# IONIQ6000/av1-go

Hardware: AMD Instinct MI355X
Metric: encoded 4K30 frames/sec (whole node) at fixed QP; PSNR-Y delta vs libaom (higher is better)
Workload: dtype u16

## Files before the change

### av1-go_amd/csrc/av1_entropy_kernels.hip

```cpp
#include <string.h>
#include <vector>
#include "av1_ops_cdfs.hpp"
#include "av1_ops32.hpp"
#include "av1mi_internal.hpp"

namespace av1mi {
using namespace av1ops;

struct Av1EntLaunch {
  FrameView fv;
  int nframes, sbr_n, sbc_n;
  BlockInfo *info;
  op_t *ops; uint32_t ops_cap;
  uint32_t *grouped; uint32_t grouped_cap;
  uint16_t *slot_total, *slot_base;
  uint16_t *rec;
  uint32_t *nops;
  uint8_t *slots; uint32_t slot_cap;
  uint32_t *tile_size;
  uint64_t *tile_off;
  uint32_t *status;
  uint8_t *out; uint64_t out_cap;
  const uint16_t *cdf_image; int cdf_words;
  SlotTable tab;
  const uint16_t *cdf_image32; SlotTable tab32;
  const uint8_t *lr_on_frame;
  int sb_rows32, band, nslots;
};

template <int kKey = -1> __device__ __forceinline__ FrameView frame_view(const Av1EntLaunch &L, int f) {
  FrameView v = L.fv;
  const long nb = (long)v.w8 * v.h8;
  if (kKey < 0 ? v.key != 0 : kKey != 0) { v.y_mode += nb * f; v.uv_mode += nb * f; }
  else { v.mv += nb * 2 * f; v.skip += nb * f; }
  v.lev_y += nb * 64 * f; v.lev_u += nb * 16 * f; v.lev_v += nb * 16 * f;
  v.info = L.info + nb * f;
  if (L.lr_on_frame) for (int p = 0; p < 3; p++) v.lr_on[p] = v.lr_on[p] && L.lr_on_frame[f * 3 + p];
  return v;
}

__global__ __launch_bounds__(256) void k_av1_info(Av1EntLaunch L) {
  const long nb = (long)L.fv.w8 * L.fv.h8, i = (long)blockIdx.x * 256 + threadIdx.x;
  if (i >= nb * L.nframes) return;
  const int f = (int)(i / nb), b = (int)(i - (long)f * nb);
  const FrameView v = frame_view(L, f);
  BlockInfo o = {};
  block_summary(v, b, &o);
  if (!v.key) inter_mode_decision(v, b / v.w8, b % v.w8, &o);
  L.info[nb * f + b] = o;
}

constexpr int kReplaySlots = (S_MAX + 1) / 2;
struct TokLds {
  union {
    struct { uint8_t cnt[S_MAX * kBlocksPerTile]; alignas(16) uint8_t mag[kBlocksPerTile * kMagBytes]; } p1;
    uint16_t pos[kReplaySlots * kBlocksPerTile];
  };
  uint16_t total[S_MAX], base[S_MAX];
  ScanTables scan;
};

__global__ __launch_bounds__(64) __attribute__((amdgpu_waves_per_eu(2, 8))) void k_av1_tokens(Av1EntLaunch L) {
  const int tiles = L.sbr_n * L.sbc_n, t = blockIdx.x, f = t / tiles, tt = t - f * tiles, sbr = tt / L.sbc_n, sbc = tt - sbr * L.sbc_n;
  if (sbr < L.sb_rows32) return;
  const FrameView v = frame_view(L, f);
  const int zi = threadIdx.x, nslots = v.key ? S_KEY_END : S_INTER_END;
  __shared__ TokLds S;
  {
    uint32_t *m = reinterpret_cast<uint32_t *>(S.p1.cnt);
    for (int i = zi; i < S_MAX * kBlocksPerTile / 4; i += 64) m[i] = 0;
    if (zi == 0) fill_scan_tables(&S.scan);
  }
  __syncthreads();
  const int below = tiles - L.sb_rows32 * L.sbc_n;
  uint16_t *rec = L.rec + (((size_t)f * below + (tt - (tiles - below))) * kBlocksPerTile + zi) * kBlockRecords;
  const TokScratch ts = { S.p1.mag + zi * kMagBytes, &S.scan };
  Sink k = { rec, S.p1.cnt, zi, 0, 0, false };
  tok_block(v, k, ts, sbr, sbc, zi);
  int x = k.n;
#pragma unroll
  for (int d = 1; d < 64; d <<= 1) {
    const int y = __shfl_up(x, d, 64);
    if (zi >= d) x += y;
  }
  const int total = __shfl(x, 63, 64), first = x - k.n;
  if ((uint32_t)total > L.ops_cap || __any(k.overflow)) {
    if (zi == 0) { atomicOr(L.status, 1u); L.nops[t] = 0; }
    for (int sl = zi; sl < S_MAX; sl += 64) L.slot_total[(size_t)t * S_MAX + sl] = 0;
    return;
  }
  if (zi == 0) L.nops[t] = (uint32_t)total;
  __syncthreads();
  constexpr int kOwn = (S_MAX + 63) / 64;
  uint32_t c[kOwn][kBlocksPerTile / 4];
#pragma unroll
  for (int q = 0; q < kOwn; q++) {
    const int sl = zi + 64 * q;
    int sum = 0;
#pragma unroll
    for (int w = 0; w < kBlocksPerTile / 4; w++) {
      const uint32_t u = sl < nslots ? reinterpret_cast<const uint32_t *>(S.p1.cnt)[sl * (kBlocksPerTile / 4) + w] : 0u;
      c[q][w] = u;
      sum = (int)__builtin_amdgcn_sad_u8(u, 0u, (unsigned)sum);
    }
    if (sl < S_MAX) S.total[sl] = (uint16_t)sum;
  }
  __syncthreads();
  {
    int mine = 0;
    for (int q = 0; q < 4; q++) { const int sl = 4 * zi + q; if (sl < nslots) mine += (S.total[sl] + kListAlign - 1) & ~(kListAlign - 1); }
    int inc = mine;
#pragma unroll
    for (int d = 1; d < 64; d <<= 1) {
      const int y = __shfl_up(inc, d, 64);
      if (zi >= d) inc += y;
    }
    int run = inc - mine;
    for (int q = 0; q < 4; q++) { const int sl = 4 * zi + q; if (sl < nslots) { S.base[sl] = (uint16_t)run; run += (S.total[sl] + kListAlign - 1) & ~(kListAlign - 1); } }
  }
  __syncthreads();
#pragma unroll
  for (int q = 0; q < kOwn; q++) {
    const int sl = zi + 64 * q;
    if (sl >= S_MAX) continue;
    const bool on = sl < nslots;
    L.slot_total[(size_t)t * S_MAX + sl] = on ? S.total[sl] : (uint16_t)0;
    L.slot_base[(size_t)t * S_MAX + sl] = on ? S.base[sl] : (uint16_t)0;
  }
  op_t *list = L.ops + (size_t)t * L.ops_cap;
  uint32_t *grouped = L.grouped + (size_t)t * L.grouped_cap;
#pragma unroll
  for (int half = 0; half < 2; half++) {
    const int lo = half * kReplaySlots, hi = lo + kReplaySlots;
    if (half) __syncthreads();
#pragma unroll
    for (int q = 0; q < kOwn; q++) {
      const int sl = zi + 64 * q;
      if (sl < lo || sl >= hi || sl >= nslots) continue;
      int run = S.base[sl];
#pragma unroll
      for (int w = 0; w < kBlocksPerTile / 4; w++) {
        const uint32_t u = c[q][w];
        const int p0 = run, p1 = p0 + (int)(u & 0xFF), p2 = p1 + (int)((u >> 8) & 0xFF), p3 = p2 + (int)((u >> 16) & 0xFF);
        run = p3 + (int)(u >> 24);
        uint32_t *d = reinterpret_cast<uint32_t *>(S.pos + (sl - lo) * kBlocksPerTile + 4 * w);
        d[0] = (uint32_t)p0 | ((uint32_t)p1 << 16); d[1] = (uint32_t)p2 | ((uint32_t)p3 << 16);
      }
    }
    __syncthreads();
    __threadfence_block();
    replay_block<kBlocksPerTile>(rec, k.nrec, S.pos, zi, first, list, grouped, lo, hi, half == 0);
  }
}

struct Wave32 {
  template <class T> using Var = LaneVar<T, 1>;
  template <class F> __device__ __forceinline__ void each(F f) { f((int)threadIdx.x); __syncthreads(); }
  __device__ __forceinline__ int scan(Var<int> &v) {
    const int lane = (int)threadIdx.x, x = v.v[0];
    int inc = x;
#pragma unroll
    for (int d = 1; d < 64; d <<= 1) {
      const int y = __shfl_up(inc, d, 64);
      if (lane >= d) inc += y;
    }
    v.v[0] = inc - x;
    return __shfl(inc, 63, 64);
  }
  __device__ __forceinline__ int first(Var<int> &v) { return __shfl(v.v[0], 0, 64); }
};
__global__ __launch_bounds__(64) void k_av1_tokens32(Av1EntLaunch L) {
  __shared__ Tile32Mem S;
  const int tiles = L.sbr_n * L.sbc_n, band = L.sb_rows32 * L.sbc_n, f = blockIdx.x / band, tt = blockIdx.x - f * band, sbr = tt / L.sbc_n, sbc = tt - sbr * L.sbc_n;
  const size_t t = (size_t)f * tiles + tt;
  const FrameView v = frame_view<1>(L, f);
  Wave32 w;
  const int n = tok_tile32(w, S, v, sbr, sbc, L.ops + t * L.ops_cap, L.ops_cap, L.grouped + t * L.grouped_cap, L.slot_total + t * S_MAX, L.slot_base + t * S_MAX);
  if (threadIdx.x == 0) {
    if (n < 0) atomicOr(L.status, 1u);
    L.nops[t] = n < 0 ? 0u : (uint32_t)n;
  }
}

__global__ __launch_bounds__(64) void k_av1_chains(Av1EntLaunch L, int ntiles_all, int ngroups) {
  const int xcd = blockIdx.x & 7, j = blockIdx.x >> 3, nslots = L.nslots;
  const int g = (j / nslots) * 8 + xcd, sl = j - (j / nslots) * nslots, lane = threadIdx.x, t = g * 64 + lane;
  if (g >= ngroups) return;
  __shared__ __attribute__((aligned(16))) uint16_t s_big[64 * 16];
  const int n = L.tab.nsym[sl], off = L.tab.off[sl];
  int cnt = 0, base = 0;
  bool mine = t < ntiles_all;
  if (mine && L.band) { const int tiles = L.sbr_n * L.sbc_n, sbr = (t % tiles) / L.sbc_n; mine = (sbr < L.sb_rows32) == (L.band == 1); }
  if (mine) { cnt = L.slot_total[(size_t)t * S_MAX + sl]; base = L.slot_base[(size_t)t * S_MAX + sl]; }
  if (!__any(cnt > 0)) return;
  const size_t tt = t < ntiles_all ? (size_t)t : 0;
  op_t *list = L.ops + tt * L.ops_cap;
  const uint32_t *grouped = L.grouped + tt * L.grouped_cap + base;
  if (n <= 4) {
    const uint32_t *iw = reinterpret_cast<const uint32_t *>(L.cdf_image) + (off >> 1);
    uint64_t cdf = (uint64_t)iw[0] | ((uint64_t)iw[1] << 32);
    const uint4 *g4 = reinterpret_cast<const uint4 *>(grouped);
    const uint4 z = make_uint4(0, 0, 0, 0);
    uint4 c0 = cnt > 0 ? g4[0] : z, c1 = cnt > 4 ? g4[1] : z, c2 = cnt > 8 ? g4[2] : z, c3 = cnt > 12 ? g4[3] : z;
    auto four = [&](const uint4 &v, int e) {
      if (e < cnt) list[v.x >> 4] = small_step(cdf, (int)(v.x & 15), n);
      if (e + 1 < cnt) list[v.y >> 4] = small_step(cdf, (int)(v.y & 15), n);
      if (e + 2 < cnt) list[v.z >> 4] = small_step(cdf, (int)(v.z & 15), n);
      if (e + 3 < cnt) list[v.w >> 4] = small_step(cdf, (int)(v.w & 15), n);
    };
#pragma unroll 1
    for (int e = 0; e < cnt; e += 16) {
      const uint4 *nx = g4 + (e >> 2) + 4;
      const uint4 n0 = e + 16 < cnt ? nx[0] : z, n1 = e + 20 < cnt ? nx[1] : z, n2 = e + 24 < cnt ? nx[2] : z, n3 = e + 28 < cnt ? nx[3] : z;
      four(c0, e); four(c1, e + 4); four(c2, e + 8); four(c3, e + 12);
      c0 = n0; c1 = n1; c2 = n2; c3 = n3;
    }
  } else {
    uint16_t *cdf = s_big + lane * 16;
    {
      const uint4 *iw = reinterpret_cast<const uint4 *>(L.cdf_image + off);
      uint4 *d = reinterpret_cast<uint4 *>(cdf);
      d[0] = iw[0];
      d[1] = n > 8 ? iw[1] : make_uint4(0, 0, 0, 0);
    }
#pragma unroll 1
    for (int e = 0; e < cnt; e++) {
      const uint32_t v = grouped[e];
      const int s = (int)(v & 15);
      list[v >> 4] = s >= kSplitHorz ? split_tuple(cdf, s) : big_step(cdf, s, n);
    }
  }
}

constexpr int kRingOps = 64, kLaneWords = kRingOps * 2 + Coder::kStage + 8;

__global__ __launch_bounds__(64) void k_av1_code(Av1EntLaunch L, int ntiles_all) {
  __shared__ __attribute__((aligned(16))) uint16_t s_lane[64 * kLaneWords];
  const int lane = threadIdx.x, t = blockIdx.x * 64 + lane;
  const bool live = t < ntiles_all;
  uint32_t *ring = reinterpret_cast<uint32_t *>(s_lane + lane * kLaneWords);
  Coder c;
  c.init(L.slots + (size_t)(live ? t : 0) * L.slot_cap, (int)L.slot_cap, s_lane + lane * kLaneWords + kRingOps * 2);
  const int n = live ? (int)L.nops[t] : 0;
  const uint4 *ops4 = reinterpret_cast<const uint4 *>(L.ops + (size_t)(live ? t : 0) * L.ops_cap);
  uint4 r0, r1, r2, r3, r4, r5, r6, r7;
  r0 = r1 = r2 = r3 = r4 = r5 = r6 = r7 = make_uint4(0, 0, 0, 0);
  int w = 0;
  bool pend = false;
  auto request = [&]() {
    const uint4 *p = ops4 + (w >> 2);
    if (w < n) r0 = p[0];
    if (w + 4 < n) r1 = p[1];
    if (w + 8 < n) r2 = p[2];
    if (w + 12 < n) r3 = p[3];
    if (w + 16 < n) r4 = p[4];
    if (w + 20 < n) r5 = p[5];
    if (w + 24 < n) r6 = p[6];
    if (w + 28 < n) r7 = p[7];
    pend = w < n;
  };
  auto take = [&]() {
    uint4 *q = reinterpret_cast<uint4 *>(ring + (w & 32));
    q[0] = r0; q[1] = r1; q[2] = r2; q[3] = r3; q[4] = r4; q[5] = r5; q[6] = r6; q[7] = r7;
    w += 32;
  };
  request();
  if (pend) { take(); request(); }
  int i = 0, lit_left = 0;
  uint32_t op = ring[0], op_next = ring[1], op_next2 = ring[2];
  for (;;) {
    if (!__any(lit_left > 0 || i < n)) break;
    if (__any((pend && w - i < 24) || c.ns >= Coder::kStage - 8)) {
      if (pend && w - i <= 32) { take(); request(); }
      c.spill();
    }
#pragma unroll
    for (int q = 0; q < 8; q++) {
      if (lit_left > 0 || i < n) {
        const uint32_t fetched = ring[(i + 3) & (kRingOps - 1)];
        uint32_t tup = op;
        if (lit_left == 0 && (op >> 31)) lit_left = (int)((op >> 27) & 15);
        if (lit_left > 0) {
          lit_left--;
          tup = (op >> lit_left) & 1 ? (1u << 19) | (256u << 9) : (2u << 19) | (512u << 9) | 256u;
        }
        c.encode_tuple(tup);
        if (lit_left == 0) { i++; op = op_next; op_next = op_next2; op_next2 = fetched; }
      }
    }
  }
  if (!live) return;
  int sz = n ? c.finish() : -1;
  if (sz < 0) { if (n) atomicOr(L.status, 2u); sz = 0; }
  L.tile_size[t] = (uint32_t)sz;
}

__global__ __launch_bounds__(1024) void k_av1_scan(Av1EntLaunch L, int ntiles_all) {
  __shared__ uint64_t part[1024];
  const int tid = threadIdx.x, per = (ntiles_all + 1023) / 1024, i0 = tid * per, i1 = min(i0 + per, ntiles_all);
  uint64_t s = 0;
  for (int i = i0; i < i1; i++) s += L.tile_size[i];
  part[tid] = s;
  __syncthreads();
  for (int d = 1; d < 1024; d <<= 1) {
    const uint64_t y = tid >= d ? part[tid - d] : 0;
    __syncthreads();
    part[tid] += y;
    __syncthreads();
  }
  uint64_t run = part[tid] - s;
  for (int i = i0; i < i1; i++) { L.tile_off[i] = run; run += L.tile_size[i]; }
  if (tid == 1023) {
    L.tile_off[ntiles_all] = part[1023];
    if (part[1023] > L.out_cap) atomicOr(L.status, 4u);
  }
}
__global__ __launch_bounds__(64) void k_av1_gather(Av1EntLaunch L) {
  const int t = blockIdx.x;
  const uint32_t n = L.tile_size[t];
  const uint64_t off = L.tile_off[t];
  if (off + n > L.out_cap) return;
  const uint8_t *src = L.slots + (size_t)t * L.slot_cap;
  uint8_t *dst = L.out + off;
  const uint32_t head = min(n, (uint32_t)((16 - (reinterpret_cast<uintptr_t>(dst) & 15)) & 15)), body = (n - head) >> 4, tail0 = head + (body << 4);
  if (threadIdx.x < head) dst[threadIdx.x] = src[threadIdx.x];
  for (uint32_t i = threadIdx.x; i < body; i += 64) {
    uint4 v;
    __builtin_memcpy(&v, src + head + 16 * i, 16);
    *reinterpret_cast<uint4 *>(dst + head + 16 * i) = v;
  }
  if (tail0 + threadIdx.x < n) dst[tail0 + threadIdx.x] = src[tail0 + threadIdx.x];
}

hipError_t launch_av1_front(av1mi_ctx *ctx, const Av1EntLaunch &L, hipStream_t s) {
  const long nb = (long)L.fv.w8 * L.fv.h8 * L.nframes;
  const int ntiles_all = L.sbr_n * L.sbc_n * L.nframes, ngroups = (ntiles_all + 63) / 64;
  ProfToken t = ctx_prof_begin(ctx, AV1MI_K_ENTROPY_TOKENS, s);
  hipLaunchKernelGGL(k_av1_info, dim3((unsigned)((nb + 255) / 256)), dim3(256), 0, s, L);
  if (L.sb_rows32 < L.sbr_n) hipLaunchKernelGGL(k_av1_tokens, dim3((unsigned)ntiles_all), dim3(64), 0, s, L);
  if (L.sb_rows32) hipLaunchKernelGGL(k_av1_tokens32, dim3((unsigned)(L.sb_rows32 * L.sbc_n * L.nframes)), dim3(64), 0, s, L);
  ctx_prof_end(ctx, t, s);
  t = ctx_prof_begin(ctx, AV1MI_K_ENTROPY_CHAINS, s);
  Av1EntLaunch C = L;
  C.nslots = L.fv.key ? S_KEY_END : S_INTER_END; C.band = L.sb_rows32 ? 2 : 0;
  if (L.sb_rows32 < L.sbr_n) hipLaunchKernelGGL(k_av1_chains, dim3((unsigned)(((ngroups + 7) / 8) * 8 * C.nslots)), dim3(64), 0, s, C, ntiles_all, ngroups);
  if (L.sb_rows32) {
    C.nslots = K_END; C.band = 1; C.tab = L.tab32; C.cdf_image = L.cdf_image32;
    hipLaunchKernelGGL(k_av1_chains, dim3((unsigned)(((ngroups + 7) / 8) * 8 * C.nslots)), dim3(64), 0, s, C, ntiles_all, ngroups);
  }
  ctx_prof_end(ctx, t, s);
  return hipGetLastError();
}
hipError_t launch_av1_back(av1mi_ctx *ctx, const Av1EntLaunch &L, hipStream_t s) {
  const int ntiles_all = L.sbr_n * L.sbc_n * L.nframes;
  ProfToken t = ctx_prof_begin(ctx, AV1MI_K_ENTROPY, s);
  hipLaunchKernelGGL(k_av1_code, dim3((unsigned)((ntiles_all + 63) / 64)), dim3(64), 0, s, L, ntiles_all);
  ctx_prof_end(ctx, t, s);
  t = ctx_prof_begin(ctx, AV1MI_K_ENTROPY_PACK, s);
  hipLaunchKernelGGL(k_av1_scan, dim3(1), dim3(1024), 0, s, L, ntiles_all);
  hipLaunchKernelGGL(k_av1_gather, dim3((unsigned)ntiles_all), dim3(64), 0, s, L);
  ctx_prof_end(ctx, t, s);
  return hipGetLastError();
}

}

struct av1mi_av1ent_state {
  void *info = nullptr, *ops[2] = { nullptr, nullptr }, *nops[2] = { nullptr, nullptr }, *grouped = nullptr, *slot_tb = nullptr, *rec = nullptr, *slots = nullptr, *tile_off = nullptr, *status = nullptr;
  size_t info_b = 0, ops_b[2] = { 0, 0 }, nops_b[2] = { 0, 0 }, grouped_b = 0, slot_tb_b = 0, rec_b = 0, slots_b = 0, off_b = 0;
  hipEvent_t lists_ready[2] = { nullptr, nullptr }, lists_free[2] = { nullptr, nullptr };
  bool free_recorded[2] = { false, false };
  unsigned long jobs = 0;
  av1mi::Av1EntLaunch pending[2];
  uint64_t *pending_total[2] = { nullptr, nullptr };
  bool pending_valid[2] = { false, false };
  size_t last_tiles = 0;
  uint16_t *d_image[2][4] = {};
  uint16_t *d_image32[4] = {};
  av1ops::SlotTable tab32;
  int image_words[2] = { 0, 0 };
  av1ops::SlotTable tab[2];
};

namespace {
int grow(av1mi_ctx *ctx, void **p, size_t *have, size_t need) {
  if (*have >= need) return AV1MI_OK;
  if (*p) (void)hipFree(*p);
  *p = nullptr; *have = 0;
  if (hipMalloc(p, need) != hipSuccess) return av1mi::ctx_fail(ctx, AV1MI_E_NOMEM, "AV1 entropy scratch: hipMalloc(%zu) failed", need);
  *have = need;
  return AV1MI_OK;
}
}

extern "C" {

uint32_t av1mi_av1_entropy_ops_per_tile(void) { return 32768; }
uint32_t av1mi_av1_entropy_slot_bytes(void) { return 16384; }

}

int av1mi::av1_entropy_front(av1mi_ctx *ctx, const av1mi_av1_entropy_job *j, hipStream_t front, int *ticket) {
  if (!ctx || !ticket) return AV1MI_E_INVAL;
  *ticket = -1;
  if (!j) return av1mi::ctx_fail(ctx, AV1MI_E_INVAL, "null job");
  if (hipSetDevice(av1mi::ctx_device(ctx)) != hipSuccess) return av1mi::ctx_fail(ctx, AV1MI_E_DEVICE, "hipSetDevice failed");
  if (j->width <= 0 || j->height <= 0 || (j->width & 7) || (j->height & 7) || j->width > 4096 || j->height > 4096)
    return av1mi::ctx_fail(ctx, AV1MI_E_INVAL, "frame %dx%d must be a multiple of 8, at most 4096x4096", j->width, j->height);
  if (j->nframes < 0 || j->nframes > 4096 || j->base_q_idx < 1 || j->base_q_idx > 255) return av1mi::ctx_fail(ctx, AV1MI_E_INVAL, "bad nframes / base_q_idx");
  const void *need[] = { j->d_lev_y, j->d_lev_u, j->d_lev_v, j->d_out, j->d_tile_size, j->d_total, j->key ? (const void *)j->d_modes_y : (const void *)j->d_mvs,
                         j->key ? (const void *)j->d_modes_uv : (const void *)j->d_skip };
  for (const void *p : need) if (!p) return av1mi::ctx_fail(ctx, AV1MI_E_INVAL, "null device pointer");
  if (j->nframes == 0) return AV1MI_OK;
  av1mi_av1ent_state *st = av1mi::ctx_av1ent(ctx);
  if (!st) return av1mi::ctx_fail(ctx, AV1MI_E_NOMEM, "AV1 entropy state");
  const int key = j->key ? 1 : 0, qcat = av1ops::q_category(j->base_q_idx);
  if (!st->d_image[key][qcat]) {
    av1ops::SlotTable tab;
    const std::vector<uint16_t> img = av1ops::default_slot_image(key != 0, qcat, &tab);
    st->tab[key] = tab; st->image_words[key] = tab.words;
    if (hipMalloc((void **)&st->d_image[key][qcat], img.size() * 2) != hipSuccess ||
        hipMemcpy(st->d_image[key][qcat], img.data(), img.size() * 2, hipMemcpyHostToDevice) != hipSuccess)
      return av1mi::ctx_fail(ctx, AV1MI_E_DEVICE, "uploading the default CDF image failed");
  }
  if (j->key_rows32 && (!key || (j->key_rows32 & 63) || j->key_rows32 > j->height || (j->width & 31)))
    return av1mi::ctx_fail(ctx, AV1MI_E_INVAL, "key_rows32 %d: whole superblock rows of a key frame whose width is a multiple of 32", j->key_rows32);
  if (j->key_rows32 && !st->d_image32[qcat]) {
    const std::vector<uint16_t> img = av1ops::default_slot_image_k32(qcat, &st->tab32);
    if (hipMalloc((void **)&st->d_image32[qcat], img.size() * 2) != hipSuccess ||
        hipMemcpy(st->d_image32[qcat], img.data(), img.size() * 2, hipMemcpyHostToDevice) != hipSuccess)
      return av1mi::ctx_fail(ctx, AV1MI_E_DEVICE, "uploading the default CDF image failed");
  }
  av1mi::Av1EntLaunch L;
  memset(&L, 0, sizeof(L));
  L.sb_rows32 = j->key_rows32 / 64;
  if (j->key_rows32) { L.tab32 = st->tab32; L.cdf_image32 = st->d_image32[qcat]; }
  L.fv.w8 = j->width / 8; L.fv.h8 = j->height / 8; L.fv.key = key;
  L.fv.y_mode = j->d_modes_y; L.fv.uv_mode = j->d_modes_uv; L.fv.mv = j->d_mvs; L.fv.skip = j->d_skip;
  L.fv.lev_y = j->d_lev_y; L.fv.lev_u = j->d_lev_u; L.fv.lev_v = j->d_lev_v;
  for (int p = 0; p < 3; p++) {
    L.fv.lr_on[p] = j->lr_on[p] != 0;
    const int vh = j->visible_height ? j->visible_height : j->height, vw = j->visible_width ? j->visible_width : j->width;
    const int ph = p ? (vh + 1) / 2 : vh, pw = p ? (vw + 1) / 2 : vw;
    L.fv.lr_rows[p] = (ph + 32) / 64 > 1 ? (ph + 32) / 64 : 1; L.fv.lr_cols[p] = (pw + 32) / 64 > 1 ? (pw + 32) / 64 : 1;
  }
  memcpy(L.fv.lr_unit[0], j->lr_unit_y, 8); memcpy(L.fv.lr_unit[1], j->lr_unit_uv, 8);
  L.nframes = j->nframes; L.sbr_n = (L.fv.h8 + 7) / 8; L.sbc_n = (L.fv.w8 + 7) / 8;
  const size_t nb = (size_t)L.fv.w8 * L.fv.h8 * j->nframes, nt = (size_t)L.sbr_n * L.sbc_n * j->nframes;
  L.ops_cap = av1mi_av1_entropy_ops_per_tile(); L.slot_cap = av1mi_av1_entropy_slot_bytes();
  L.grouped_cap = L.ops_cap + av1ops::kListAlign * av1ops::S_MAX;
  const int par = (int)(st->jobs++ & 1);
  st->last_tiles = nt;
  int rc;
  if ((rc = grow(ctx, &st->info, &st->info_b, nb * sizeof(av1ops::BlockInfo))) ||
      (rc = grow(ctx, &st->ops[par], &st->ops_b[par], nt * L.ops_cap * sizeof(av1ops::op_t))) || (rc = grow(ctx, &st->nops[par], &st->nops_b[par], nt * 4)) ||
      (rc = grow(ctx, &st->grouped, &st->grouped_b, nt * L.grouped_cap * sizeof(uint32_t))) ||
      (rc = grow(ctx, &st->slot_tb, &st->slot_tb_b, nt * av1ops::S_MAX * 4)) ||
      (rc = grow(ctx, &st->rec, &st->rec_b, (size_t)(L.sbr_n - L.sb_rows32) * L.sbc_n * j->nframes * av1ops::kBlocksPerTile * av1ops::kBlockRecords * sizeof(uint16_t))) ||
      (rc = grow(ctx, &st->slots, &st->slots_b, nt * L.slot_cap)) || (rc = grow(ctx, &st->tile_off, &st->off_b, (nt + 1) * 8)))
    return rc;
  L.info = (av1ops::BlockInfo *)st->info; L.ops = (av1ops::op_t *)st->ops[par]; L.nops = (uint32_t *)st->nops[par]; L.grouped = (uint32_t *)st->grouped;
  L.slot_total = (uint16_t *)st->slot_tb; L.slot_base = L.slot_total + nt * av1ops::S_MAX; L.rec = (uint16_t *)st->rec; L.slots = (uint8_t *)st->slots;
  L.tile_off = (uint64_t *)st->tile_off;
  L.tile_size = j->d_tile_size; L.out = j->d_out; L.out_cap = j->out_cap;
  L.status = (uint32_t *)(j->d_total + 1);
  L.cdf_image = st->d_image[key][qcat]; L.cdf_words = st->image_words[key]; L.tab = st->tab[key];
  L.lr_on_frame = j->d_lr_on;
#define E_HIP(call) do { const hipError_t e_ = (call); if (e_ != hipSuccess) return av1mi::ctx_fail(ctx, AV1MI_E_DEVICE, "%s: %s", #call, hipGetErrorString(e_)); } while (0)
  for (hipEvent_t *ev : { &st->lists_ready[par], &st->lists_free[par] }) if (!*ev) E_HIP(hipEventCreateWithFlags(ev, hipEventDisableTiming));
  if (st->free_recorded[par]) E_HIP(hipStreamWaitEvent(front, st->lists_free[par], 0));
  E_HIP(hipMemsetAsync(j->d_total, 0, 16, front));
  E_HIP(av1mi::launch_av1_front(ctx, L, front));
  E_HIP(hipEventRecord(st->lists_ready[par], front));
  st->pending[par] = L; st->pending_total[par] = j->d_total; st->pending_valid[par] = true;
  *ticket = par;
  return AV1MI_OK;
}

int av1mi::av1_entropy_back(av1mi_ctx *ctx, int ticket, hipStream_t back) {
  if (!ctx || ticket < 0 || ticket > 1) return AV1MI_E_INVAL;
  av1mi_av1ent_state *st = av1mi::ctx_av1ent(ctx);
  if (!st || !st->pending_valid[ticket]) return av1mi::ctx_fail(ctx, AV1MI_E_INVAL, "no entropy job pending under this ticket");
  const av1mi::Av1EntLaunch &L = st->pending[ticket];
  const size_t nt = (size_t)L.sbr_n * L.sbc_n * L.nframes;
  E_HIP(hipStreamWaitEvent(back, st->lists_ready[ticket], 0));
  E_HIP(av1mi::launch_av1_back(ctx, L, back));
  E_HIP(hipMemcpyAsync(st->pending_total[ticket], L.tile_off + nt, 8, hipMemcpyDeviceToDevice, back));
  E_HIP(hipEventRecord(st->lists_free[ticket], back)); st->free_recorded[ticket] = true;
  st->pending_valid[ticket] = false;
#undef E_HIP
  return AV1MI_OK;
}

int av1mi::av1_entropy_submit(av1mi_ctx *ctx, const av1mi_av1_entropy_job *j, hipStream_t front, hipStream_t back) {
  int ticket = -1;
  const int rc = av1_entropy_front(ctx, j, front, &ticket);
  if (rc != AV1MI_OK || ticket < 0) return rc;
  return av1_entropy_back(ctx, ticket, back);
}

extern "C" {

int av1mi_av1_entropy_encode_on(av1mi_ctx *ctx, const av1mi_av1_entropy_job *j, void *stream_handle) {
  if (!ctx) return AV1MI_E_INVAL;
  hipStream_t s = stream_handle ? (hipStream_t)stream_handle : av1mi::ctx_stream(ctx);
  return av1mi::av1_entropy_submit(ctx, j, s, s);
}

int av1mi_av1_entropy_encode(av1mi_ctx *ctx, const av1mi_av1_entropy_job *j) { return av1mi_av1_entropy_encode_on(ctx, j, nullptr); }

int av1mi_av1_entropy_last_list_words(av1mi_ctx *ctx, uint64_t *words) {
  if (!ctx || !words) return AV1MI_E_INVAL;
  *words = 0;
  av1mi_av1ent_state *st = av1mi::ctx_av1ent(ctx);
  if (!st || !st->jobs || !st->last_tiles) return AV1MI_OK;
  if (hipSetDevice(av1mi::ctx_device(ctx)) != hipSuccess || hipDeviceSynchronize() != hipSuccess) return av1mi::ctx_fail(ctx, AV1MI_E_DEVICE, "synchronising failed");
  std::vector<uint32_t> n(st->last_tiles);
  if (hipMemcpy(n.data(), st->nops[(st->jobs - 1) & 1], n.size() * 4, hipMemcpyDeviceToHost) != hipSuccess) return av1mi::ctx_fail(ctx, AV1MI_E_DEVICE, "reading the list sizes failed");
  for (uint32_t v : n) *words += v;
  return AV1MI_OK;
}

}

namespace av1mi {
void av1ent_free(av1mi_av1ent_state *st) {
  if (!st) return;
  for (void *p : { st->info, st->ops[0], st->ops[1], st->nops[0], st->nops[1], st->grouped, st->slot_tb, st->rec, st->slots, st->tile_off }) if (p) (void)hipFree(p);
  for (hipEvent_t ev : { st->lists_ready[0], st->lists_ready[1], st->lists_free[0], st->lists_free[1] }) if (ev) (void)hipEventDestroy(ev);
  for (auto &k : st->d_image) for (uint16_t *p : k) if (p) (void)hipFree(p);
  for (uint16_t *p : st->d_image32) if (p) (void)hipFree(p);
  delete st;
}
av1mi_av1ent_state *av1ent_new() { return new (std::nothrow) av1mi_av1ent_state(); }
}
```

### av1-go_amd/csrc/av1_ops.hpp

```cpp
#pragma once
#include <stdint.h>

#if defined(__HIPCC__)
#include <hip/hip_runtime.h>
#define AV1_HD __host__ __device__ inline
#define AV1_UNROLL _Pragma("unroll")
#define AV1_NOUNROLL _Pragma("unroll 1")
#else
#define AV1_HD inline
#define AV1_UNROLL
#define AV1_NOUNROLL
#endif

namespace av1ops {

typedef uint16_t __attribute__((may_alias)) u16a;
typedef uint32_t __attribute__((may_alias)) u32a;
typedef uint64_t __attribute__((may_alias)) u64a;

enum Slot : int {
  S_SKIP = 0,
  S_PART8 = S_SKIP + 3,
  S_PART16 = S_PART8 + 1,
  S_PART32 = S_PART16 + 4,
  S_PART64 = S_PART32 + 4,
  S_USE_WIENER = S_PART64 + 4,
  S_TXB_SKIP_Y = S_USE_WIENER + 1,
  S_TXB_SKIP_C = S_TXB_SKIP_Y + 1,
  S_EOB64_Y = S_TXB_SKIP_C + 3,
  S_EOB16_C = S_EOB64_Y + 1,
  S_EOBX_Y = S_EOB16_C + 1,
  S_EOBX_C = S_EOBX_Y + 5,
  S_DC_SIGN_Y = S_EOBX_C + 3,
  S_DC_SIGN_C = S_DC_SIGN_Y + 3,
  S_BASE_EOB_Y = S_DC_SIGN_C + 3,
  S_BASE_EOB_C = S_BASE_EOB_Y + 4,
  S_BASE_Y = S_BASE_EOB_C + 4,
  S_BASE_C = S_BASE_Y + 26,
  S_BR_Y = S_BASE_C + 26,
  S_BR_C = S_BR_Y + 21,
  S_COMMON_END = S_BR_C + 21,
  S_KF_Y_MODE = S_COMMON_END,
  S_UV_MODE = S_KF_Y_MODE + 25,
  S_ANGLE = S_UV_MODE + 13,
  S_INTRA_TX = S_ANGLE + 8,
  S_KEY_END = S_INTRA_TX + 13,
  S_IS_INTER = S_COMMON_END,
  S_SINGLE_REF = S_IS_INTER + 4,
  S_NEW_MV = S_SINGLE_REF + 6,
  S_ZERO_MV = S_NEW_MV + 6,
  S_REF_MV = S_ZERO_MV + 1,
  S_DRL = S_REF_MV + 6,
  S_MV_JOINT = S_DRL + 3,
  S_MV_COMP = S_MV_JOINT + 1,
  S_INTER_TX = S_MV_COMP + 32,
  S_INTER_END = S_INTER_TX + 1,
  S_MAX = S_KEY_END > S_INTER_END ? S_KEY_END : S_INTER_END
};
enum { MVC_CLASS = 0, MVC_CLASS0 = 1, MVC_CLASS0_FR = 2, MVC_SIGN = 4, MVC_BITS = 5, MVC_FR = 15 };

struct BandSlots {
  int use_wiener, kf_y_mode, uv_mode, angle;
  int txb_skip_y, txb_skip_c, eob_y, eob_c, eobx_y, eobx_c, dc_sign_y, dc_sign_c, base_eob_y, base_eob_c, base_y, base_c, br_y, br_c;
  int eob_y_n, eob_c_n;
};
constexpr BandSlots kSlots8 = { S_USE_WIENER, S_KF_Y_MODE, S_UV_MODE, S_ANGLE, S_TXB_SKIP_Y, S_TXB_SKIP_C, S_EOB64_Y, S_EOB16_C, S_EOBX_Y,
                                S_EOBX_C, S_DC_SIGN_Y, S_DC_SIGN_C, S_BASE_EOB_Y, S_BASE_EOB_C, S_BASE_Y, S_BASE_C, S_BR_Y, S_BR_C, 7, 5 };

template <const BandSlots &B> AV1_HD int coeff_nsym(int s) {
  if (s < B.txb_skip_y || s >= B.br_c + 21) return 0;
  if (s == B.eob_y) return B.eob_y_n;
  if (s == B.eob_c) return B.eob_c_n;
  return s < B.base_eob_y ? 2 : s < B.base_y ? 3 : 4;
}
AV1_HD int slot_nsym(int s, bool key) {
  if (const int n = coeff_nsym<kSlots8>(s)) return n;
  if (s < S_PART8) return 2;
  if (s < S_PART16) return 4;
  if (s < S_USE_WIENER) return 10;
  if (s < S_COMMON_END) return 2;
  if (key) {
    if (s < S_UV_MODE) return 13;
    if (s < S_ANGLE) return 14;
    if (s < S_INTRA_TX) return 7;
    return 7;
  }
  if (s < S_MV_JOINT) return 2;
  if (s == S_MV_JOINT) return 4;
  if (s < S_INTER_TX) {
    const int k = (s - S_MV_COMP) & 15;
    return k == MVC_CLASS ? 11 : (k == MVC_CLASS0_FR || k == MVC_CLASS0_FR + 1 || k == MVC_FR) ? 4 : 2;
  }
  return 16;
}
AV1_HD int q_category(int base_q_idx) { return base_q_idx <= 20 ? 0 : base_q_idx <= 60 ? 1 : base_q_idx <= 120 ? 2 : 3; }
AV1_HD int slot_words(int nsym) { return nsym <= 4 ? 4 : nsym <= 8 ? 8 : 16; }

typedef uint32_t op_t;
struct SlotTable { uint16_t off[S_MAX]; uint8_t nsym[(S_MAX + 3) & ~3]; int words; };
AV1_HD op_t op_lit(int n, unsigned v) { return (op_t)(0x80000000u | ((unsigned)n << 27) | (v & 0x7FFu)); }
AV1_HD op_t make_tuple(uint32_t fl, uint32_t fh, int s, int n) { return (op_t)(((unsigned)(n - s) << 19) | ((fl >> 6) << 9) | (fh >> 6)); }
enum { kBlocksPerTile = 64, kSplitHorz = 14, kSplitVert = 15, kListAlign = 4, kBlockRecords = 1024 };

struct Sink {
  uint16_t *rec;
  uint8_t *cnt;
  int zi, nrec, n;
  bool overflow;
  AV1_HD void put(unsigned r) { if (nrec < kBlockRecords) rec[nrec] = (uint16_t)r; else overflow = true; nrec++; n++; }
  AV1_HD void sym(int slot, int s) {
    put(((unsigned)slot << 4) | (unsigned)s);
    uint8_t &c = cnt[slot * kBlocksPerTile + zi];
    if (c == 255) overflow = true; else c++;
  }
  AV1_HD void split(int kind, int slot) { sym(slot, kind ? kSplitVert : kSplitHorz); }
  AV1_HD void lit(unsigned v, int nbits) {
    while (nbits > 11) { nbits -= 11; put(0x8000u | (11u << 11) | ((v >> nbits) & 0x7FFu)); }
    if (nbits > 0) put(0x8000u | ((unsigned)nbits << 11) | (v & ((1u << nbits) - 1u)));
  }
};
AV1_HD int group_positions(const uint8_t *cnt_slot, uint16_t *pos_slot, int base) {
  int run = base;
  for (int b = 0; b < kBlocksPerTile; b++) { const int c = cnt_slot[b]; pos_slot[b] = (uint16_t)run; run += c; }
  return run - base;
}
template <int kBlocks>
AV1_HD void replay_block(const uint16_t *rec, int nrec, uint16_t *pos, int blk, int first, op_t *list, uint32_t *grouped, int slot_lo = 0,
                         int slot_hi = 1 << 16, bool literals = true) {
  int n = first;
  for (int i0 = 0; i0 < nrec; i0 += 8) {
    struct alignas(16) R8 { uint32_t w[4]; } q = *reinterpret_cast<const R8 *>(rec + i0);
    AV1_UNROLL
    for (int j = 0; j < 8; j++, n++) {
      if (i0 + j >= nrec) break;
      const unsigned r = (q.w[j >> 1] >> (16 * (j & 1))) & 0xFFFFu;
      if (r & 0x8000u) { if (literals) list[n] = op_lit((int)((r >> 11) & 15), r & 0x7FFu); }
      else {
        const int sl = (int)(r >> 4);
        if (sl >= slot_lo && sl < slot_hi) { uint16_t &p = pos[(sl - slot_lo) * kBlocks + blk]; grouped[p] = ((uint32_t)n << 4) | (r & 15u); p++; }
      }
    }
  }
}

struct BlockInfo { uint8_t cul[3], dc[3], mode, flags; uint8_t num, drl; int16_t px, py; uint8_t pad[2]; };
struct FrameView {
  int w8, h8;
  int key;
  const uint8_t *y_mode, *uv_mode;
  const int16_t *mv;
  const uint8_t *skip;
  const int16_t *lev_y, *lev_u, *lev_v;
  const BlockInfo *info;
  int lr_on[3];
  int8_t lr_unit[2][8];
  int lr_rows[3], lr_cols[3];
};

AV1_HD int iabs(int v) { return v < 0 ? -v : v; }
AV1_HD int imin(int a, int b) { return a < b ? a : b; }
AV1_HD int imax(int a, int b) { return a > b ? a : b; }
AV1_HD int ilog2(unsigned v) { return 31 - __builtin_clz(v | 1u); }
AV1_HD unsigned morton8(unsigned x, unsigned y) {
  unsigned m = 0;
  for (int i = 0; i < 3; i++) m |= ((x >> i) & 1u) << (2 * i) | ((y >> i) & 1u) << (2 * i + 1);
  return m;
}
AV1_HD void demorton8(unsigned k, int *bx, int *by) {
  int x = 0, y = 0;
  for (int i = 0; i < 3; i++) { x |= ((k >> (2 * i)) & 1) << i; y |= ((k >> (2 * i + 1)) & 1) << i; }
  *bx = x; *by = y;
}

AV1_HD void block_summary(const FrameView &f, int b, BlockInfo *o) {
  const int16_t *p[3] = { f.lev_y + (long)b * 64, f.lev_u + (long)b * 16, f.lev_v + (long)b * 16 };
  const bool skip = !f.key && f.skip[b];
  for (int pl = 0; pl < 3; pl++) {
    int cul = 0;
    const int n = pl ? 16 : 64;
    for (int i = 0; i < n; i++) cul += iabs(p[pl][i]);
    o->cul[pl] = skip ? 0 : (uint8_t)imin(cul, 63);
    o->dc[pl] = skip ? 0 : (uint8_t)(p[pl][0] < 0 ? 1 : p[pl][0] > 0 ? 2 : 0);
  }
}

struct MvCand { int16_t x, y; int weight; };
struct MvStack { MvCand st[8]; int num, new_ctx, ref_ctx; };

AV1_HD void mv_stack(const FrameView &f, int r8, int c8, bool use_flags, MvStack *S) {
  const int r0 = r8 & ~7, c0 = c8 & ~7, r1 = imin(r0 + 8, f.h8), c1 = imin(c0 + 8, f.w8);
  int num = 0, new_count = 0;
  bool found = false;
  MvCand *st = S->st;
  auto add = [&](int r, int c, bool count_new) {
    if (r < r0 || r >= r1 || c < c0 || c >= c1) return;
    const int nb = r * f.w8 + c;
    const int16_t mx = f.mv[2 * nb], my = f.mv[2 * nb + 1];
    if (count_new && use_flags && (f.info[nb].flags & 1)) new_count++;
    found = true;
    int i = 0;
    for (; i < num; i++) if (st[i].x == mx && st[i].y == my) break;
    if (i < num) st[i].weight += 4;
    else if (num < 8) { st[num].x = mx; st[num].y = my; st[num].weight = 4; num++; }
  };
  add(r8 - 1, c8, true);
  const bool above0 = found; found = false;
  add(r8, c8 - 1, true);
  const bool left0 = found; found = false;
  {
    const int tr = r8 - 1, tc = c8 + 1;
    if (tr >= r0 && tc < c1 && morton8(tc & 7, tr & 7) < morton8(c8 & 7, r8 & 7)) add(tr, tc, true);
  }
  bool above = above0 || found; found = false;
  const int close = (above ? 1 : 0) + (left0 ? 1 : 0);
  const int num_nearest = num, num_new = new_count;
  for (int i = 0; i < num_nearest; i++) st[i].weight += 640;
  add(r8 - 1, c8 - 1, false);
  above = above || found; found = false;
  bool left = left0;
  add(r8 - 2, c8, false); above = above || found; found = false;
  add(r8, c8 - 2, false); left = left || found; found = false;
  add(r8 - 3, c8, false); above = above || found; found = false;
  add(r8, c8 - 3, false); left = left || found; found = false;
  const int total = (above ? 1 : 0) + (left ? 1 : 0);
  for (int pass = 0; pass < 2; pass++) {
    const int a = pass ? num_nearest : 0, bnd = pass ? num : num_nearest;
    for (int len = bnd; len > a;) {
      int nr = a;
      for (int i = a + 1; i < len; i++)
        if (st[i - 1].weight < st[i].weight) { const MvCand t = st[i - 1]; st[i - 1] = st[i]; st[i] = t; nr = i; }
      len = nr;
    }
  }
  if (close == 0) { S->new_ctx = imin(total, 1); S->ref_ctx = total; }
  else if (close == 1) { S->new_ctx = 3 - imin(num_new, 1); S->ref_ctx = 2 + total; }
  else { S->new_ctx = 5 - imin(num_new, 1); S->ref_ctx = 5; }
  const int mi_r = r8 * 2, mi_c = c8 * 2, border = 128 + 2 * 4 * 8;
  const int top = -(mi_r * 32) - border, bottom = (f.h8 * 2 - 2 - mi_r) * 32 + border;
  const int lft = -(mi_c * 32) - border, right = (f.w8 * 2 - 2 - mi_c) * 32 + border;
  for (int i = 0; i < num; i++) {
    st[i].y = (int16_t)imin(imax(st[i].y, top), bottom);
    st[i].x = (int16_t)imin(imax(st[i].x, lft), right);
  }
  for (int i = num; i < 2; i++) { st[i].x = st[i].y = 0; st[i].weight = 0; }
  S->num = num;
}
AV1_HD void inter_mode_decision(const FrameView &f, int r8, int c8, BlockInfo *o) {
  MvStack S;
  mv_stack(f, r8, c8, false, &S);
  const int b = r8 * f.w8 + c8, mx = f.mv[2 * b], my = f.mv[2 * b + 1];
  int mode = 3, ref_idx = 0;
  if (S.st[0].x == mx && S.st[0].y == my) mode = 0;
  else {
    for (int i = 1; i < imax(S.num, 2) && i < 4; i++)
      if (S.st[i].x == mx && S.st[i].y == my) { mode = 1; ref_idx = i; break; }
    if (mode == 3 && mx == 0 && my == 0) mode = 2;
  }
  if (mode == 3) {
    const int nsel = imin(S.num, 3);
    long best = -1;
    for (int i = 0; i < imax(nsel, 1); i++) {
      const long c = iabs(mx - S.st[i].x) + iabs(my - S.st[i].y);
      if (best < 0 || c < best) { best = c; ref_idx = i; }
    }
  }
  o->mode = (uint8_t)(mode | (ref_idx << 2));
  o->flags = (uint8_t)(mode == 3);
  o->num = (uint8_t)S.num;
  int drl = 0;
  for (int i = 0; i < 4; i++) if (i < imax(S.num, 2) && S.st[i].weight >= 640) drl |= 1 << i;
  o->drl = (uint8_t)drl;
  const int pred = S.num <= 1 ? 0 : ref_idx;
  o->px = S.st[pred].x; o->py = S.st[pred].y;
}

template <class K> AV1_HD void tok_subexp(K &k, int num_syms, int kk, int v) {
  int i = 0, mk = 0;
  for (;;) {
    const int b2 = i ? kk + i - 1 : kk, a = 1 << b2;
    if (num_syms <= mk + 3 * a) {
      const int n = num_syms - mk, x = v - mk, w = ilog2((unsigned)n) + 1, m = (1 << w) - n;
      if (x < m) k.lit((unsigned)x, w - 1);
      else { k.lit((unsigned)((x + m) >> 1), w - 1); k.lit((unsigned)((x + m) & 1), 1); }
      return;
    }
    const int more = v >= mk + a;
    k.lit((unsigned)more, 1);
    if (!more) { k.lit((unsigned)(v - mk), b2); return; }
    i++; mk += a;
  }
}
AV1_HD int tok_recenter(int r, int v) { return v > 2 * r ? v : v >= r ? 2 * (v - r) : 2 * (r - v) - 1; }
template <class K> AV1_HD void tok_signed_subexp_ref(K &k, int v, int low, int high, int kk, int r) {
  const int mx = high - low;
  v -= low; r -= low;
  tok_subexp(k, mx, kk, (r << 1) <= mx ? tok_recenter(r, v) : tok_recenter(mx - 1 - r, mx - 1 - v));
}
template <const BandSlots &B, class K> AV1_HD void tok_lr(const FrameView &f, K &k, int sbr, int sbc) {
  const int mi_r = sbr * 16, mi_c = sbc * 16;
  for (int p = 0; p < 3; p++) {
    if (!f.lr_on[p]) continue;
    const int ss = p ? 1 : 0, us = 64;
    const int row0 = (mi_r * (4 >> ss) + us - 1) / us, row1 = imin(((mi_r + 16) * (4 >> ss) + us - 1) / us, f.lr_rows[p]);
    const int col0 = (mi_c * (4 >> ss) + us - 1) / us, col1 = imin(((mi_c + 16) * (4 >> ss) + us - 1) / us, f.lr_cols[p]);
    const int8_t *u = f.lr_unit[p ? 1 : 0];
    for (int ur = row0; ur < row1; ur++)
      for (int uc = col0; uc < col1; uc++) {
        k.sym(B.use_wiener, u[0] == 1);
        if (u[0] != 1) continue;
        const int kmin[3] = { -5, -23, -17 }, kmax[3] = { 10, 8, 46 }, kk[3] = { 1, 2, 3 }, mid[3] = { 3, -7, 15 };
        for (int pass = 0; pass < 2; pass++)
          for (int j = p ? 1 : 0; j < 3; j++) tok_signed_subexp_ref(k, u[1 + pass * 3 + j], kmin[j], kmax[j] + 1, kk[j], mid[j]);
      }
  }
}
template <const BandSlots &B, class K> AV1_HD void tok_kf_modes(K &k, int ym, int uvm, int above, int left) {
  static const uint8_t kCtx[13] = { 0, 1, 2, 3, 4, 4, 4, 4, 3, 0, 1, 2, 0 };
  k.sym(B.kf_y_mode + kCtx[above] * 5 + kCtx[left], ym);
  if (ym >= 1 && ym <= 8) k.sym(B.angle + ym - 1, 3);
  k.sym(B.uv_mode + ym, uvm);
  if (uvm >= 1 && uvm <= 8) k.sym(B.angle + uvm - 1, 3);
}
AV1_HD void tok_partition_prefix(const FrameView &f, Sink &k, int sbr, int sbc, int bx, int by) {
  const int mi_rows = f.h8 * 2, mi_cols = f.w8 * 2;
  for (int bsize = 64; bsize >= 16; bsize >>= 1) {
    const int n8 = bsize >> 3;
    if ((bx & (n8 - 1)) || (by & (n8 - 1))) continue;
    const int r = (sbr * 8 + by) * 2, c = (sbc * 8 + bx) * 2, half = bsize >> 3;
    const bool has_rows = r + half < mi_rows, has_cols = c + half < mi_cols;
    const bool au = by > 0, al = bx > 0;
    const int slot = (bsize == 16 ? S_PART16 : bsize == 32 ? S_PART32 : S_PART64) + (al ? 2 : 0) + (au ? 1 : 0);
    if (has_rows && has_cols) k.sym(slot, 3);
    else if (has_cols) k.split(0, slot);
    else if (has_rows) k.split(1, slot);
  }
  k.sym(S_PART8, 0);
}

struct ScanTables { uint8_t s4[16], s8[64], i4[16], i8[64]; };
AV1_HD void fill_scan_tables(ScanTables *t) {
  for (int N = 4; N <= 8; N += 4) {
    uint8_t *o = N == 4 ? t->s4 : t->s8;
    int k = 0;
    for (int d = 0; d < 2 * N - 1; d++)
      for (int i = 0; i <= d; i++) {
        const int r = (d & 1) ? i : d - i, c = d - r;
        if (r < N && c < N) o[k++] = (uint8_t)(r * N + c);
      }
    uint8_t *inv = N == 4 ? t->i4 : t->i8;
    for (int i = 0; i < N * N; i++) inv[o[i]] = (uint8_t)i;
  }
}
enum { kMagStride = 10, kMagBytes = 100 };
struct TokScratch { uint8_t *mag; const ScanTables *scan; };

template <int N, bool kBytes = (N <= 8)> struct MagMap;
template <int N> struct MagMap<N, true> {
  enum { LG = N == 4 ? 2 : 3, MS = kMagStride };
  uint8_t *mag;
  const uint8_t *scan, *iscan;
  AV1_HD MagMap(const TokScratch &ts) : mag(ts.mag), scan(N == 4 ? ts.scan->s4 : ts.scan->s8), iscan(N == 4 ? ts.scan->i4 : ts.scan->i8) {}
  AV1_HD int load(const int16_t *lev) {
    for (int i = 0; i < (N + 2) * MS / 4; i++) reinterpret_cast<u32a *>(mag)[i] = 0;
    int eob = 0;
    for (int r = 0; r < N * N / 8; r++) {
      struct alignas(16) L8 { int16_t v[8]; } q = *reinterpret_cast<const L8 *>(lev + 8 * r);
      for (int j = 0; j < 8; j++) {
        const int pos = 8 * r + j, v = q.v[j], a = iabs(v);
        if (v) eob = imax(eob, iscan[pos] + 1);
        mag[(pos >> LG) * MS + (pos & (N - 1))] = (uint8_t)((a > 15 ? 15 : a) | (v < 0 ? 128 : 0));
      }
    }
    return eob;
  }
  AV1_HD int pos(int c) const { return scan[c]; }
  AV1_HD int at(int i) const { return mag[i] & 15; }
  AV1_HD int neg(int p) const { return mag[(p >> LG) * MS + (p & (N - 1))] >> 7; }
};

template <int N, const BandSlots &B, class K>
AV1_HD void tok_coeffs_lead(K &k, bool chroma, int eob, int above_cul, int above_dc, int left_cul, int left_dc, int tx_slot, int tx_sym) {
  k.sym(chroma ? B.txb_skip_c + ((above_cul | above_dc) != 0) + ((left_cul | left_dc) != 0) : B.txb_skip_y, eob == 0);
  if (!eob) return;
  if (tx_slot >= 0) k.sym(tx_slot, tx_sym);
  const int eob_pt = eob < 3 ? eob : ilog2((unsigned)(eob - 1)) + 2;
  k.sym(chroma ? B.eob_c : B.eob_y, eob_pt - 1);
  if (eob_pt >= 3) {
    const int off = eob - ((1 << (eob_pt - 2)) + 1), shift = eob_pt - 3;
    k.sym((chroma ? B.eobx_c : B.eobx_y) + eob_pt - 3, (off >> shift) & 1);
    if (shift > 0) k.lit((unsigned)(off & ((1 << shift) - 1)), shift);
  }
}
template <int N, const BandSlots &B, class K, class M_>
AV1_HD void tok_coeffs_pass1(K &k, const M_ &M, bool chroma, const int16_t *lev, int eob, int c_hi, int c_lo) {
  const int nc = N * N, LG = M.LG, MS = M.MS;
  const int base_eob = chroma ? B.base_eob_c : B.base_eob_y, base = chroma ? B.base_c : B.base_y, br = chroma ? B.br_c : B.br_y;
  for (int c = c_hi; c >= c_lo; c--) {
    const int pos = M.pos(c), row = pos >> LG, col = pos & (N - 1), at = row * MS + col;
    const int m0 = M.at(at), m1 = M.at(at + 1), m2 = M.at(at + 2), mb = M.at(at + MS), md = M.at(at + MS + 1), mbb = M.at(at + 2 * MS);
    int a = m0;
    if (a == 15) a = iabs(lev[pos]);
    if (c == eob - 1) {
      k.sym(base_eob + (c == 0 ? 0 : c <= nc / 8 ? 1 : c <= nc / 4 ? 2 : 3), imin(a, 3) - 1);
    } else {
      const int mm = imin(m1, 3) + imin(mb, 3) + imin(md, 3) + imin(m2, 3) + imin(mbb, 3);
      int bctx = imin((mm + 1) >> 1, 4);
      if (pos == 0) bctx = 0;
      else bctx += row + col < 2 ? 1 : row + col < 4 ? 6 : 21;
      k.sym(base + bctx, imin(a, 3));
    }
    if (a > 2) {
      int mm = m1 + mb + md;
      mm = imin((mm + 1) >> 1, 6);
      const int rctx = pos == 0 ? mm : (row < 2 && col < 2) ? mm + 7 : mm + 14;
      int rem = a - 3;
      for (int i = 0; i < 4; i++) {
        const int q = imin(rem, 3);
        k.sym(br + rctx, q);
        rem -= q;
        if (q < 3) break;
      }
    }
  }
}
template <int N, const BandSlots &B, class K, class M_>
AV1_HD void tok_coeffs_pass2(K &k, const M_ &M, bool chroma, const int16_t *lev, int above_dc, int left_dc, int c_lo, int c_hi) {
  const int LG = M.LG, MS = M.MS;
  for (int c = c_lo; c < c_hi; c++) {
    const int pos = M.pos(c), m = M.at((pos >> LG) * MS + (pos & (N - 1)));
    if (!m) continue;
    const int neg = M.neg(pos);
    if (c == 0) {
      const int sg = (above_dc == 2) - (above_dc == 1) + (left_dc == 2) - (left_dc == 1);
      k.sym((chroma ? B.dc_sign_c : B.dc_sign_y) + (sg < 0 ? 1 : sg > 0 ? 2 : 0), neg);
    } else {
      k.lit((unsigned)neg, 1);
    }
    if (m == 15) {
      const int a = iabs(lev[pos]);
      if (a > 14) {
        const unsigned x = (unsigned)(a - 14);
        const int len = ilog2(x) + 1;
        k.lit(0, len - 1);
        k.lit(x, len);
      }
    }
  }
}
template <int N, const BandSlots &B, class K, class TS>
AV1_HD void tok_coeffs(K &k, const TS &ts, bool chroma, const int16_t *lev, int above_cul, int above_dc, int left_cul, int left_dc, int tx_slot,
                       int tx_sym) {
  MagMap<N> M(ts);
  const int eob = M.load(lev);
  tok_coeffs_lead<N, B>(k, chroma, eob, above_cul, above_dc, left_cul, left_dc, tx_slot, tx_sym);
  if (!eob) return;
  tok_coeffs_pass1<N, B>(k, M, chroma, lev, eob, eob - 1, 0);
  tok_coeffs_pass2<N, B>(k, M, chroma, lev, above_dc, left_dc, 0, eob);
}

AV1_HD void tok_mv_comp(Sink &k, int comp, int diff) {
  const int base = S_MV_COMP + comp * 16;
  k.sym(base + MVC_SIGN, diff < 0);
  const int off = iabs(diff) - 1, cls = (off >> 3) < 2 ? 0 : ilog2((unsigned)(off >> 3));
  k.sym(base + MVC_CLASS, cls);
  if (cls == 0) {
    k.sym(base + MVC_CLASS0, off >> 3);
    k.sym(base + MVC_CLASS0_FR + (off >> 3), (off >> 1) & 3);
  } else {
    const int o = off - (2 << (cls + 2)), d = o >> 3;
    for (int i = 0; i < cls; i++) k.sym(base + MVC_BITS + i, (d >> i) & 1);
    k.sym(base + MVC_FR, (o >> 1) & 3);
  }
}

AV1_HD void tok_block(const FrameView &f, Sink &k, const TokScratch &ts, int sbr, int sbc, int zi) {
  int bx, by;
  demorton8((unsigned)zi, &bx, &by);
  const int r8 = sbr * 8 + by, c8 = sbc * 8 + bx;
  if (r8 >= f.h8 || c8 >= f.w8) return;
  if (zi == 0) tok_lr<kSlots8>(f, k, sbr, sbc);
  tok_partition_prefix(f, k, sbr, sbc, bx, by);
  const int b = r8 * f.w8 + c8;
  const bool au = by > 0, al = bx > 0;
  const BlockInfo zero = {};
  const BlockInfo ia = au ? f.info[b - f.w8] : zero, il = al ? f.info[b - 1] : zero;
  const int skip = f.key ? 0 : f.skip[b];
  k.sym(S_SKIP + (au && !f.key ? f.skip[b - f.w8] : 0) + (al && !f.key ? f.skip[b - 1] : 0), skip);
  int ym = 0;
  if (f.key) {
    ym = f.y_mode[b];
    tok_kf_modes<kSlots8>(k, ym, f.uv_mode[b], au ? f.y_mode[b - f.w8] : 0, al ? f.y_mode[b - 1] : 0);
  } else {
    k.sym(S_IS_INTER + 0, 1);
    const int rctx = (au || al) ? 1 : 0;
    k.sym(S_SINGLE_REF + rctx * 3 + 0, 0);
    k.sym(S_SINGLE_REF + rctx * 3 + 1, 0);
    k.sym(S_SINGLE_REF + rctx * 3 + 2, 0);
    const BlockInfo me = f.info[b];
    const int mode = me.mode & 3, ref_idx = me.mode >> 2, num = me.num;
    const int mx = f.mv[2 * b], my = f.mv[2 * b + 1];
    const int close = (au ? 1 : 0) + (al ? 1 : 0);
    int num_new = (au ? ia.flags & 1 : 0) + (al ? il.flags & 1 : 0);
    if (au && bx < 7 && c8 + 1 < f.w8 && morton8((unsigned)bx + 1, (unsigned)by - 1) < morton8((unsigned)bx, (unsigned)by)) num_new += f.info[b - f.w8 + 1].flags & 1;
    const int new_ctx = close == 0 ? 0 : close == 1 ? 3 - imin(num_new, 1) : 5 - imin(num_new, 1);
    const int ref_ctx = close == 0 ? 0 : close == 1 ? 3 : 5;
    k.sym(S_NEW_MV + new_ctx, mode != 3);
    if (mode != 3) {
      k.sym(S_ZERO_MV, mode != 2);
      if (mode != 2) k.sym(S_REF_MV + ref_ctx, mode == 1);
    }
    auto drl_ctx = [&](int i) {
      const bool a = (me.drl >> i) & 1, c = (me.drl >> (i + 1)) & 1;
      return a && c ? 0 : a ? 1 : !c ? 2 : 0;
    };
    if (mode == 3) {
      for (int i = 0; i < 2; i++)
        if (num > i + 1) {
          k.sym(S_DRL + drl_ctx(i), ref_idx != i);
          if (ref_idx == i) break;
        }
      const int dx = mx - me.px, dy = my - me.py;
      k.sym(S_MV_JOINT, (dx ? 1 : 0) + (dy ? 2 : 0));
      if (dy) tok_mv_comp(k, 0, dy);
      if (dx) tok_mv_comp(k, 1, dx);
    } else if (mode == 1) {
      for (int i = 1; i < 3; i++)
        if (num > i + 1) {
          k.sym(S_DRL + drl_ctx(i), ref_idx != i);
          if (ref_idx == i) break;
        }
    }
  }
  if (skip) return;
  tok_coeffs<8, kSlots8>(k, ts, false, f.lev_y + (long)b * 64, ia.cul[0], ia.dc[0], il.cul[0], il.dc[0], f.key ? S_INTRA_TX + ym : S_INTER_TX, f.key ? 1 : 7);
  AV1_NOUNROLL
  for (int p = 1; p < 3; p++)
    tok_coeffs<4, kSlots8>(k, ts, true, (p == 1 ? f.lev_u : f.lev_v) + (long)b * 16, ia.cul[p], ia.dc[p], il.cul[p], il.dc[p], -1, 0);
}

template <class F> AV1_HD void build_slot_table(int n, F nsym, SlotTable *t) {
  int o = 0;
  for (int s = 0; s < S_MAX; s++) {
    if (s < n) {
      t->nsym[s] = (uint8_t)nsym(s);
      const int w = slot_words(t->nsym[s]), al = w < 8 ? 4 : 8;
      o = (o + al - 1) & ~(al - 1);
      t->off[s] = (uint16_t)o;
      o += w;
    } else { t->nsym[s] = 2; t->off[s] = 0; }
  }
  t->words = (o + 7) & ~7;
}
AV1_HD void build_slot_table(bool key, SlotTable *t) { build_slot_table(key ? S_KEY_END : S_INTER_END, [key](int s) { return slot_nsym(s, key); }, t); }

#ifdef AV1_CODER_STATS
static long long coder_stat_carries = 0;
#endif
struct Coder {
  enum { kStage = 32 };
  uint64_t low;
  uint32_t rng;
  int nb;
  uint8_t *out;
  uint16_t *stage;
  int pos, cap, ns;
  bool overflow;
  AV1_HD void init(uint8_t *o, int c, uint16_t *st) { low = 0; rng = 0x8000; nb = -1; out = o; stage = st; pos = 0; cap = c; ns = 0; overflow = false; }
  AV1_HD void carry_back() {
    for (int k = ns; k-- > 0;) { const uint16_t v = (uint16_t)(stage[k] + 1); stage[k] = v; if (v) return; }
    for (int i = pos; i-- > 0;) if (++out[i] != 0) return;
  }
  AV1_HD bool stage_full() const { return ns >= kStage - 1; }
  AV1_HD void spill() {
    if (pos + 2 * ns > cap) { overflow = true; pos += 2 * ns; ns = 0; return; }
    for (int k = 0; k < ns; k++) { const uint32_t v = stage[k]; *reinterpret_cast<uint16_t *>(out + pos + 2 * k) = (uint16_t)((v >> 8) | (v << 8)); }
    pos += 2 * ns; ns = 0;
  }
  AV1_HD void flush16() {
    nb -= 16;
    const uint32_t w = (uint32_t)(low >> (16 + nb));
    if ((w >> 16) && !overflow) {
#ifdef AV1_CODER_STATS
      coder_stat_carries++;
#endif
      carry_back();
    }
    stage[ns++] = (uint16_t)w;
    low &= ((uint64_t)1 << (16 + nb)) - 1;
  }
  AV1_HD void encode(uint32_t fl, uint32_t fh, int s, int n) {
    const uint32_t r = rng, v = (((r >> 8) * (fh >> 6)) >> 1) + 4u * (uint32_t)(n - 1 - s);
    const uint32_t u = fl < 32768u ? (((r >> 8) * (fl >> 6)) >> 1) + 4u * (uint32_t)(n - s) : r;
    low += r - u;
    const uint32_t nr = u - v;
    const int d = 15 - ilog2(nr);
    rng = nr << d; low <<= d; nb += d;
    if (nb >= 32) flush16();
  }
  AV1_HD void encode_tuple(op_t t) {
    const uint32_t fl6 = (t >> 9) & 1023u, fh6 = t & 511u, dl = (t >> 19) & 31u;
    const uint32_t r = rng, v = (((r >> 8) * fh6) >> 1) + 4u * (dl - 1u);
    const uint32_t u = fl6 < 512u ? (((r >> 8) * fl6) >> 1) + 4u * dl : r;
    low += r - u;
    const uint32_t nr = u - v;
    const int d = 15 - ilog2(nr);
    rng = nr << d; low <<= d; nb += d;
    if (nb >= 32) flush16();
  }
  AV1_HD void bit(int b) { encode(b ? 16384u : 32768u, b ? 0u : 16384u, b, 2); }
  AV1_HD int finish() {
    uint64_t e = ((low + 0x3FFF) & ~(uint64_t)0x3FFF) | 0x4000;
    if (nb >= 0 && (e >> (16 + nb))) { if (!overflow) carry_back(); e &= ((uint64_t)1 << (16 + nb)) - 1; }
    spill();
    int top = 15 + nb;
    while (top >= 14) {
      uint8_t byte = 0;
      for (int q = 7; q >= 0 && top >= 14; q--, top--) byte |= (uint8_t)(((e >> top) & 1) << q);
      if (pos < cap) out[pos] = byte; else overflow = true;
      pos++;
    }
    return overflow ? -1 : pos;
  }
};

AV1_HD uint32_t adapt(uint32_t x, bool below, int rate) {
  const uint32_t m = 0u - (uint32_t)below, d = ((x ^ m) + (m & 32769u)) >> rate;
  return x - ((d ^ m) - m);
}

AV1_HD op_t small_step(uint64_t &w, int s, int n) {
  const uint32_t x0 = (uint32_t)w & 0xFFFFu, x1 = (uint32_t)w >> 16, x2 = (uint32_t)(w >> 32) & 0xFFFFu, cnt = (uint32_t)(w >> 48);
  const uint32_t fl = s == 0 ? 32768u : s == 1 ? x0 : s == 2 ? x1 : x2;
  const uint32_t fh = s == n - 1 ? 0u : s == 0 ? x0 : s == 1 ? x1 : x2;
  const int rate = 3 + (cnt > 15) + (cnt > 31) + (n >= 4 ? 2 : 1);
  const uint32_t y0 = adapt(x0, 0 < s, rate), y1 = adapt(x1, 1 < s, rate), y2 = adapt(x2, 2 < s, rate), ncnt = cnt + (cnt < 32);
  w = (uint64_t)(y0 | (y1 << 16)) | ((uint64_t)(y2 | (ncnt << 16)) << 32);
  return make_tuple(fl, fh, s, n);
}

AV1_HD op_t big_step(uint16_t *v, int s, int n) {
  const int nd = n > 8 ? 8 : 4;
  u32a *d = reinterpret_cast<u32a *>(v);
  uint32_t w[8];
  AV1_UNROLL
  for (int k = 0; k < 8; k++) w[k] = k < nd ? d[k] : 0u;
  const uint32_t fl = s ? v[s - 1] : 32768u, fh = s == n - 1 ? 0u : v[s];
  const uint32_t cnt = (nd == 8 ? w[7] : w[3]) >> 16;
  const int rate = 3 + (cnt > 15) + (cnt > 31) + 2;
  AV1_UNROLL
  for (int k = 0; k < 8; k++) {
    if (k >= nd) continue;
    uint32_t lo = adapt(w[k] & 0xFFFFu, 2 * k < s, rate), hi = adapt(w[k] >> 16, 2 * k + 1 < s, rate);
    if (k == nd - 1) hi = cnt + (cnt < 32);
    d[k] = lo | (hi << 16);
  }
  return make_tuple(fl, fh, s, n);
}

AV1_HD op_t split_tuple(const uint16_t *p, int kind) {
  const uint32_t p1 = p[0] - p[1], p2 = p[1] - p[2], p3 = p[2] - p[3], p4 = p[3] - p[4], p5 = p[4] - p[5], p6 = p[5] - p[6], p7 = p[6] - p[7],
                 p8 = p[7] - p[8], p9 = p[8];
  return make_tuple(kind == kSplitHorz ? p2 + p3 + p4 + p6 + p7 + p9 : p1 + p3 + p4 + p5 + p6 + p8, 0, 1, 2);
}

AV1_HD void run_chain(const uint16_t *init, int n, const uint32_t *g, int cnt, op_t *list) {
  if (n <= 4) {
    uint64_t w = (uint64_t)init[0] | ((uint64_t)init[1] << 16) | ((uint64_t)init[2] << 32) | ((uint64_t)init[3] << 48);
    for (int k = 0; k < cnt; k++) list[g[k] >> 4] = small_step(w, (int)(g[k] & 15), n);
    return;
  }
  alignas(16) uint16_t v[16];
  for (int i = 0; i < 16; i++) v[i] = i < slot_words(n) ? init[i] : 0;
  for (int k = 0; k < cnt; k++) {
    const int s = (int)(g[k] & 15);
    list[g[k] >> 4] = s >= kSplitHorz ? split_tuple(v, s) : big_step(v, s, n);
  }
}

AV1_HD void code_word(Coder &c, op_t e) {
  if (e >> 31) { for (int i = (int)((e >> 27) & 15) - 1; i >= 0; i--) { c.bit((e >> i) & 1); if (c.stage_full()) c.spill(); } }
  else { c.encode_tuple(e); if (c.stage_full()) c.spill(); }
}

}
```

### av1-go_amd/csrc/gop_session.hip

```cpp
#include <math.h>
#include <stdio.h>
#include <stdlib.h>
#include <string.h>
#include <new>
#include <vector>
#include "av1mi_internal.hpp"
#include "quality.hpp"

namespace {

int lf_level_from_q(int ac_q, int bd, bool key) {
  long g;
  if (bd == 8) g = key ? ((long)ac_q * 17563 - 421574 + (1 << 17)) >> 18 : ((long)ac_q * 6017 + 650707 + (1 << 17)) >> 18;
  else g = ((long)ac_q * 20723 + 4060632 + (1 << 19)) >> 20;
  return (int)(g < 0 ? 0 : g > 63 ? 63 : g);
}
void frame_params(int q, int bd, int frame_type, av1mi_frame_params *p) {
  memset(p, 0, sizeof(*p));
  const int ac_q = av1mi_ac_q(q, bd), q8 = ac_q >> (bd - 8);
  p->frame_type = frame_type; p->base_q_idx = q;
  const int lvl = lf_level_from_q(ac_q, bd, frame_type == 0);
  p->lf_level[0] = p->lf_level[1] = p->lf_level[2] = p->lf_level[3] = lvl;
  p->lf_sharpness = 0;
  p->cdef_damping = 3 + (q >> 6);
  {
    const float x = (float)q8, x2 = x * x;
    auto fit = [&](float a, float b, float c, int hi) { const int v = (int)lroundf(x2 * a + x * b + c); return v < 0 ? 0 : v > hi ? hi : v; };
    int y1, y2, c1, c2;
    if (frame_type == 0) {
      y1 = fit(0.0000033731974f, 0.008070594f, 0.0187634f, 15); y2 = fit(0.0000029167343f, 0.0027798624f, 0.0079405f, 3);
      c1 = fit(-0.0000130790995f, 0.012892405f, -0.00748388f, 15); c2 = fit(0.0000032651783f, 0.00035520183f, 0.00228092f, 3);
    } else {
      y1 = fit(-0.0000023593946f, 0.0068615186f, 0.02709886f, 15); y2 = fit(-0.00000057629734f, 0.0013993345f, 0.03831067f, 3);
      c1 = fit(-0.0000007095069f, 0.0034628846f, 0.00887099f, 15); c2 = fit(0.00000023874085f, 0.00028223585f, 0.05576307f, 3);
    }
    p->cdef_y = (uint8_t)(y1 << 2 | y2); p->cdef_uv = (uint8_t)(c1 << 2 | c2);
  }
  p->lr_unit_size = 64;
  static const int8_t wy[8] = { 1, 3, -7, 15, 3, -7, 15, 0 }, wc[8] = { 1, 0, -7, 15, 0, -7, 15, 0 };
  memcpy(p->lr_unit_y, wy, 8); memcpy(p->lr_unit_uv, wc, 8);
}

enum { kSlots = 3, kFallbacksToHostMode = 3 };

struct Plane { int ss = 0, w = 0, h = 0, vw = 0, vh = 0; size_t n = 0, bytes = 0; };

struct Slot {
  void *h_in[3] = { nullptr, nullptr, nullptr }, *d_in[3] = { nullptr, nullptr, nullptr };
  void *d_pre[3] = { nullptr, nullptr, nullptr };
  void *d_src[3] = { nullptr, nullptr, nullptr };
  void *d_lev[3] = { nullptr, nullptr, nullptr }, *h_lev[3] = { nullptr, nullptr, nullptr };
  void *d_modes[2] = { nullptr, nullptr }, *h_modes[2] = { nullptr, nullptr };
  void *d_mv = nullptr, *h_mv = nullptr, *d_skip = nullptr, *h_skip = nullptr;
  hipEvent_t uploaded = nullptr, kernel_done = nullptr, filters_done = nullptr, downloaded = nullptr;
  bool upload_pending = false, kernel_pending = false;
  void *d_lr_on = nullptr, *h_lr_on = nullptr;
  int frame_type = 0;
  int q = 0;
  av1mi_frame_params params{};
  void *h_ent_out = nullptr, *d_tile_size = nullptr, *h_tile_size = nullptr, *d_total = nullptr, *h_total = nullptr;
  hipEvent_t ent_done = nullptr;
  bool ent_pending = false;
  bool symbols_down = false;
  int ent_ticket = -1;
  void *h_quality = nullptr;
  hipEvent_t quality_done = nullptr;
};

}

struct av1mi_gop {
  av1mi_ctx *ctx = nullptr;
  av1mi_gop_config cfg{};
  Plane plane[3];
  size_t nb = 0, bps = 1;
  int fmt = AV1MI_INPUT_PLANAR;
  int stages = 0;
  bool chroma_stage = false, luma_through = false;
  int src_bd = 8;
  av1mi::ScalePlan *scale = nullptr;
  size_t fed_ny = 0;
  size_t in_bytes[3] = {}, pre_bytes[3] = {};
  hipStream_t up = nullptr, down = nullptr;
  Slot slot[kSlots];
  void *d_rec[3] = {}, *d_dbl[3] = {}, *d_cdef[3] = {}, *d_ref[3] = {};
  void *d_mi[3][2] = {};
  int key32 = 0, key_rows32 = 0;
  int key_modes_band = 0, key_modes_stride = 0;
  void *d_cdef_sb[2] = {}, *d_lr[2] = {}, *d_zero_skip = nullptr;
  void *d_lr_scratch = nullptr;
  void *d_me = nullptr;
  void *d_quality_scratch = nullptr;
  int vw = 0, vh = 0;
  int last = 0;
  av1mi_frame_params params[2];
  int next_q = 0;
  int mi_q[3] = {}, cdef_q[2] = {};
  size_t ent_cap = 0; int tiles = 0;
  long submitted = 0, collected = 0;
  long fallbacks = 0;
  bool symbols_always = false;
  int gop_pos = 0;
  bool acquired = false;
  int coder_streams = 0;
  int intra_open_loop = 0;
  std::vector<void *> dev_allocs, host_allocs;
};

namespace {

#define G_HIP(expr)                                                                                          \
  do {                                                                                                       \
    hipError_t e_ = (expr);                                                                                  \
    if (e_ != hipSuccess) return av1mi::ctx_fail(g->ctx, AV1MI_E_DEVICE, "%s: %s", #expr, hipGetErrorString(e_)); \
  } while (0)
#define G_TRY(expr)                              \
  do {                                           \
    int rc_ = (expr);                            \
    if (rc_ != AV1MI_OK) return rc_;             \
  } while (0)

int dev_alloc(av1mi_gop *g, void **p, size_t bytes) {
  G_HIP(hipMalloc(p, bytes ? bytes : 8));
  g->dev_allocs.push_back(*p);
  return AV1MI_OK;
}
int host_alloc(av1mi_gop *g, void **p, size_t bytes) {
  G_HIP(hipHostMalloc(p, bytes ? bytes : 8, hipHostMallocDefault));
  g->host_allocs.push_back(*p);
  return AV1MI_OK;
}

int slot_buffers(av1mi_gop *g, Slot &s) {
  const av1mi_gop_config &c = g->cfg;
  const int S = c.segments;
  for (int p = 0; p < 3; p++) {
    const Plane &P = g->plane[p];
    if (g->in_bytes[p]) G_TRY(host_alloc(g, &s.h_in[p], g->in_bytes[p]));
    G_TRY(dev_alloc(g, &s.d_src[p], P.bytes));
    const bool through = g->luma_through && p == 0;
    if (!g->stages || (through && g->stages == 1)) s.d_in[p] = s.d_src[p];
    else if (g->in_bytes[p]) G_TRY(dev_alloc(g, &s.d_in[p], g->in_bytes[p]));
    if (g->stages == 2 && !through) G_TRY(dev_alloc(g, &s.d_pre[p], g->pre_bytes[p]));
    if (c.gpu_entropy != 1) G_TRY(host_alloc(g, &s.h_lev[p], P.n * 2));
    G_TRY(dev_alloc(g, &s.d_lev[p], P.n * 2));
  }
  for (int k = 0; k < 2; k++) { G_TRY(host_alloc(g, &s.h_modes[k], g->nb)); G_TRY(dev_alloc(g, &s.d_modes[k], g->nb)); }
  G_TRY(host_alloc(g, &s.h_mv, g->nb * 4)); G_TRY(dev_alloc(g, &s.d_mv, g->nb * 4));
  G_TRY(host_alloc(g, &s.h_skip, g->nb)); G_TRY(dev_alloc(g, &s.d_skip, g->nb));
  for (hipEvent_t *e : { &s.uploaded, &s.kernel_done, &s.filters_done, &s.downloaded }) G_HIP(hipEventCreateWithFlags(e, hipEventDisableTiming));
  G_TRY(dev_alloc(g, &s.d_lr_on, (size_t)S * 3 + 4)); G_TRY(host_alloc(g, &s.h_lr_on, (size_t)S * 3));
  if (c.gpu_entropy) {
    G_TRY(host_alloc(g, &s.h_ent_out, g->ent_cap));
    G_TRY(dev_alloc(g, &s.d_tile_size, (size_t)g->tiles * S * 4)); G_TRY(host_alloc(g, &s.h_tile_size, (size_t)g->tiles * S * 4));
    G_TRY(dev_alloc(g, &s.d_total, 16)); G_TRY(host_alloc(g, &s.h_total, 16));
    G_HIP(hipEventCreateWithFlags(&s.ent_done, hipEventDisableTiming));
  }
  if (c.quality_stats) {
    G_TRY(host_alloc(g, &s.h_quality, (size_t)S * 3 * sizeof(av1mi_quality)));
    G_HIP(hipEventCreateWithFlags(&s.quality_done, hipEventDisableTiming));
  }
  return AV1MI_OK;
}

int side_information(av1mi_gop *g) {
  const av1mi_gop_config &c = g->cfg;
  const int w = c.width, h = c.height;
  const size_t fy = (size_t)w * h, fc = fy / 4;
  const int nsb = ((w + 63) / 64) * ((h + 63) / 64);
  auto units = [](int n) { const int u = (n + 32) / 64; return u > 1 ? u : 1; };
  const size_t uy = (size_t)units(h) * units(w), uc = (size_t)units(h / 2) * units(w / 2);
  if (c.key_block_size == 32) {
    g->key32 = 1; g->key_rows32 = (h / 64) * 64;
    g->key_modes_band = (g->key_rows32 / 8) * (w / 8);
    g->key_modes_stride = (h / 8) * (w / 8);
  }
  for (int t = 0; t < 2 + g->key32; t++) {
    if (t < 2) frame_params(c.base_q_idx, c.bit_depth, t, &g->params[t]);
    const av1mi_frame_params &P = g->params[t == 2 ? 0 : t];
    std::vector<uint32_t> mi(fy / 16, 3u | (3u << 4) | ((uint32_t)P.lf_level[0] << 8) | ((uint32_t)P.lf_level[1] << 16) | (3u << 25));
    std::vector<uint32_t> mic(fc / 16, 2u | (2u << 4) | ((uint32_t)P.lf_level[2] << 8) | ((uint32_t)P.lf_level[2] << 16) | (3u << 25));
    for (int r = 0; r < h / 4; r++) for (int cc = 0; cc < w / 4; cc++) if (4 * r >= g->vh || 4 * cc >= g->vw) mi[(size_t)r * (w / 4) + cc] = 3u | (3u << 4) | (1u << 24);
    for (int r = 0; r < h / 8; r++) for (int cc = 0; cc < w / 8; cc++) if (8 * r >= g->vh || 8 * cc >= g->vw) mic[(size_t)r * (w / 8) + cc] = 2u | (2u << 4) | (1u << 24);
    if (t == 2) {
      for (int r = 0; r < g->key_rows32 / 4; r++) for (int cc = 0; cc < w / 4; cc++) mi[(size_t)r * (w / 4) + cc] = (mi[(size_t)r * (w / 4) + cc] & ~0xFFu) | 5u | (5u << 4);
      for (int r = 0; r < g->key_rows32 / 8; r++) for (int cc = 0; cc < w / 8; cc++) mic[(size_t)r * (w / 8) + cc] = (mic[(size_t)r * (w / 8) + cc] & ~0xFFu) | 4u | (4u << 4);
    }
    G_TRY(dev_alloc(g, &g->d_mi[t][0], mi.size() * 4)); G_TRY(av1mi_upload(g->ctx, g->d_mi[t][0], mi.data(), mi.size() * 4));
    G_TRY(dev_alloc(g, &g->d_mi[t][1], mic.size() * 4)); G_TRY(av1mi_upload(g->ctx, g->d_mi[t][1], mic.data(), mic.size() * 4));
    g->mi_q[t] = c.base_q_idx;
  }
  for (int t = 0; t < 2; t++) {
    const av1mi_frame_params &P = g->params[t];
    std::vector<uint8_t> sb((size_t)nsb * 4);
    for (int i = 0; i < nsb; i++) { sb[4 * i] = P.cdef_y >> 2; sb[4 * i + 1] = P.cdef_y & 3; sb[4 * i + 2] = P.cdef_uv >> 2; sb[4 * i + 3] = P.cdef_uv & 3; }
    G_TRY(dev_alloc(g, &g->d_cdef_sb[t], sb.size())); G_TRY(av1mi_upload(g->ctx, g->d_cdef_sb[t], sb.data(), sb.size()));
    g->cdef_q[t] = c.base_q_idx;
  }
  {
    const av1mi_frame_params &P = g->params[0];
    std::vector<int8_t> lr((uy > uc ? uy : uc) * 8);
    for (size_t i = 0; i < uy; i++) memcpy(&lr[i * 8], P.lr_unit_y, 8);
    G_TRY(dev_alloc(g, &g->d_lr[0], uy * 8)); G_TRY(av1mi_upload(g->ctx, g->d_lr[0], lr.data(), uy * 8));
    for (size_t i = 0; i < uc; i++) memcpy(&lr[i * 8], P.lr_unit_uv, 8);
    G_TRY(dev_alloc(g, &g->d_lr[1], uc * 8)); G_TRY(av1mi_upload(g->ctx, g->d_lr[1], lr.data(), uc * 8));
  }
  return AV1MI_OK;
}

const char *config_error(const av1mi_gop_config *c, char (&buf)[512]) {
#define WHY(...) (snprintf(buf, sizeof(buf), __VA_ARGS__), buf)
  if (!c) return WHY("null config");
  if (c->width <= 0 || c->height <= 0 || (c->width & 7) || (c->height & 7) || c->width > 16384 || c->height > 16384)
    return WHY("frame %dx%d must be a multiple of 8", c->width, c->height);
  if (c->visible_width < 0 || c->visible_height < 0 || (c->visible_width && (c->visible_width > c->width || c->width - c->visible_width >= 8)) ||
      (c->visible_height && (c->visible_height > c->height || c->height - c->visible_height >= 8)))
    return WHY("visible size %dx%d must lie within 7 samples below the coded size %dx%d", c->visible_width, c->visible_height, c->width, c->height);
  if (c->bit_depth != 8 && c->bit_depth != 10) return WHY("bit depth %d not supported (8 or 10)", c->bit_depth);
  if (c->base_q_idx < 1 || c->base_q_idx > 255 || c->gop_length < 1 || c->segments < 1 || c->segments > 4096 || c->search_range < 0 ||
      c->search_range > 15 || c->gpu_entropy < 0 || c->gpu_entropy > 2 || c->coder_streams < 0 || c->coder_streams > 3)
    return WHY("bad base_q_idx / gop_length / segments / search_range / gpu_entropy");
  if (c->input_format < AV1MI_INPUT_PLANAR || c->input_format > AV1MI_INPUT_NV12)
    return WHY("input_format %d unknown (0 planar, 1 packed 10-bit, 2 P010, 3 NV12)", c->input_format);
  if ((c->input_format == AV1MI_INPUT_PACKED10 || c->input_format == AV1MI_INPUT_P010) && c->bit_depth != 10)
    return WHY("input_format %d (%s) needs bit_depth 10, not %d", c->input_format, c->input_format == AV1MI_INPUT_P010 ? "P010" : "packed 10-bit", c->bit_depth);
  if (c->input_format == AV1MI_INPUT_NV12 && c->bit_depth != 8) return WHY("input_format 3 (NV12) needs bit_depth 8, not %d", c->bit_depth);
  if (c->source_chroma < AV1MI_CHROMA_420 || c->source_chroma > AV1MI_CHROMA_400)
    return WHY("source_chroma %d unknown (0 4:2:0, 1 4:2:2, 2 4:4:4, 3 grey)", c->source_chroma);
  if (c->source_bit_depth != 0 && c->source_bit_depth != 8 && c->source_bit_depth != 10 && c->source_bit_depth != 12)
    return WHY("source_bit_depth %d not supported (8, 10 or 12; 0 = bit_depth)", c->source_bit_depth);
  if (const char *why = av1mi::chroma_format_error(c->source_chroma, c->source_bit_depth ? c->source_bit_depth : c->bit_depth, c->bit_depth))
    return WHY("source_bit_depth %d with bit_depth %d: %s", c->source_bit_depth, c->bit_depth, why);
  if ((c->source_chroma != AV1MI_CHROMA_420 || (c->source_bit_depth && c->source_bit_depth != c->bit_depth)) && c->input_format != AV1MI_INPUT_PLANAR)
    return WHY("a source that is not 4:2:0 at bit_depth (source_chroma %d, source_bit_depth %d) needs input_format 0 (planar), not %d", c->source_chroma,
               c->source_bit_depth, c->input_format);
  if ((c->source_width != 0) != (c->source_height != 0) || c->source_width < 0 || c->source_height < 0)
    return WHY("source size %dx%d: give both source_width and source_height, or neither", c->source_width, c->source_height);
  if (c->source_width) {
    const int tw = c->visible_width ? c->visible_width : c->width, th = c->visible_height ? c->visible_height : c->height;
    if (const char *why = av1mi::scale_geometry_error(c->source_width, c->source_height, tw, th))
      return WHY("source size %dx%d -> %dx%d: %s", c->source_width, c->source_height, tw, th, why);
  }
  if (c->key_block_size != 0 && c->key_block_size != 8 && c->key_block_size != 32) return WHY("key_block_size %d not supported (8 or 32)", c->key_block_size);
  if (c->key_block_size == 32 && (c->width & 31))
    return WHY("key_block_size 32 needs a width that is a multiple of 32");
  if (c->gpu_entropy && (c->width > 4096 || c->height > 4096)) return WHY("the AV1 tile coder takes frames up to 4096x4096");
  if ((size_t)c->height * c->segments > 65535u * 8u) return WHY("segments x height too large for one launch");
  if (c->coarse_range < 0 || c->coarse_range > 64 || (c->coarse_range & 3))
    return WHY("coarse_range %d must be 0 (off) or a multiple of 4 up to 64", c->coarse_range);
  if (c->quality_stats && ((c->visible_width ? c->visible_width : c->width) < 16 || (c->visible_height ? c->visible_height : c->height) < 16))
    return WHY("quality_stats needs a true luma size of at least 16x16");
  return nullptr;
#undef WHY
}

int setup(av1mi_gop *g) {
  const av1mi_gop_config &c = g->cfg;
  const int w = c.width, h = c.height, S = c.segments;
  g->bps = c.bit_depth == 8 ? 1 : 2;
  g->vw = c.visible_width ? c.visible_width : w; g->vh = c.visible_height ? c.visible_height : h;
  for (int p = 0; p < 3; p++) {
    Plane &P = g->plane[p];
    P.ss = p > 0;
    P.w = w >> P.ss; P.h = h >> P.ss; P.vw = (g->vw + P.ss) >> P.ss; P.vh = (g->vh + P.ss) >> P.ss;
    P.n = (size_t)P.w * P.h * S; P.bytes = P.n * g->bps;
  }
  g->nb = g->plane[0].n / 64;
  g->fmt = c.input_format;
  g->next_q = c.base_q_idx;
  const bool scaling = c.source_width != 0;
  g->src_bd = c.source_bit_depth ? c.source_bit_depth : c.bit_depth;
  g->chroma_stage = c.source_chroma != AV1MI_CHROMA_420 || g->src_bd != c.bit_depth;
  g->luma_through = g->chroma_stage && g->src_bd == c.bit_depth;
  g->stages = (g->fmt != AV1MI_INPUT_PLANAR) + g->chroma_stage + scaling;
  const int fed_w = scaling ? (c.source_width + 7) & ~7 : w, fed_rows = (scaling ? (c.source_height + 7) & ~7 : h) * S;
  g->fed_ny = (size_t)fed_w * fed_rows;
  for (int p = 0; p < 3; p++) {
    g->in_bytes[p] = g->chroma_stage ? av1mi_source_plane_bytes(c.source_chroma, g->src_bd, p, fed_w, fed_rows) : av1mi_input_plane_bytes(g->fmt, c.bit_depth, p, fed_w, fed_rows);
    g->pre_bytes[p] = av1mi_input_plane_bytes(AV1MI_INPUT_PLANAR, c.bit_depth, p, fed_w, fed_rows);
  }
  if (c.gpu_entropy) {
    g->tiles = ((w + 63) / 64) * ((h + 63) / 64);
    g->ent_cap = (size_t)w * h * S;
  }
  G_HIP(hipSetDevice(av1mi::ctx_device(g->ctx)));
  if (c.source_width) G_HIP(av1mi::scale_plan_create(c.bit_depth, c.source_width, c.source_height, g->vw, g->vh, &g->scale));
  G_HIP(hipStreamCreateWithFlags(&g->up, hipStreamNonBlocking));
  G_HIP(hipStreamCreateWithFlags(&g->down, hipStreamNonBlocking));
  for (Slot &s : g->slot) G_TRY(slot_buffers(g, s));
  for (int p = 0; p < 3; p++)
    for (void **d : { &g->d_rec[p], &g->d_dbl[p], &g->d_cdef[p], &g->d_ref[p] }) G_TRY(dev_alloc(g, d, g->plane[p].bytes));
  G_TRY(dev_alloc(g, &g->d_lr_scratch, av1mi_lr_yuv_decide_scratch_bytes(h, S)));
  if (c.coarse_range) G_TRY(dev_alloc(g, &g->d_me, av1mi::me_layout(w, h, S).bytes));
  if (c.quality_stats) G_TRY(dev_alloc(g, &g->d_quality_scratch, av1mi::quality_scratch_bytes(c.bit_depth, g->vw, g->vh, S)));
  G_TRY(dev_alloc(g, &g->d_zero_skip, g->nb));
  G_TRY(av1mi_memset(g->ctx, g->d_zero_skip, 0, g->nb));
  G_TRY(side_information(g));
  return av1mi_sync(g->ctx);
}

}

extern "C" {

int av1mi_policy_frame_params(int base_q_idx, int bit_depth, int frame_type, av1mi_frame_params *out) {
  if (!out || base_q_idx < 0 || base_q_idx > 255 || (bit_depth != 8 && bit_depth != 10) || frame_type < 0 || frame_type > 1) return AV1MI_E_INVAL;
  frame_params(base_q_idx, bit_depth, frame_type, out);
  return AV1MI_OK;
}

int av1mi_gop_open(av1mi_ctx *ctx, const av1mi_gop_config *cfg, av1mi_gop **out) {
  if (!ctx || !out) return AV1MI_E_INVAL;
  *out = nullptr;
  char why[512];
  if (config_error(cfg, why)) return av1mi::ctx_fail(ctx, AV1MI_E_INVAL, "%s", why);
  av1mi_gop *g = new (std::nothrow) av1mi_gop();
  if (!g) return AV1MI_E_NOMEM;
  g->ctx = ctx; g->cfg = *cfg;
  g->coder_streams = cfg->coder_streams;
  if (const char *e = getenv("AV1MI_INTRA_OPEN_LOOP")) g->intra_open_loop = atoi(e) ? 1 : 0;
  if (const char *e = getenv("AV1MI_CODER_STREAMS")) g->coder_streams = !strcmp(e, "side") ? 1 : !strcmp(e, "main") ? 2 : !strcmp(e, "defer") ? 3 : 0;
  const int rc = setup(g);
  if (rc != AV1MI_OK) { av1mi_gop_close(g); return rc; }
  *out = g;
  return AV1MI_OK;
}

void av1mi_gop_close(av1mi_gop *g) {
  if (!g) return;
  (void)hipSetDevice(av1mi::ctx_device(g->ctx));
  (void)av1mi_sync(g->ctx);
  if (g->up) { (void)hipStreamSynchronize(g->up); (void)hipStreamDestroy(g->up); }
  if (g->down) { (void)hipStreamSynchronize(g->down); (void)hipStreamDestroy(g->down); }
  for (Slot &s : g->slot)
    for (hipEvent_t e : { s.uploaded, s.kernel_done, s.filters_done, s.downloaded, s.ent_done, s.quality_done })
      if (e) (void)hipEventDestroy(e);
  for (void *p : g->dev_allocs) (void)hipFree(p);
  for (void *p : g->host_allocs) (void)hipHostFree(p);
  av1mi::scale_plan_destroy(g->scale);
  delete g;
}

int av1mi_gop_max_in_flight(void) { return kSlots; }

}


static int feed_source(av1mi_gop *g, Slot &s, const void *const *dev_src, const void *src[3]) {
  hipStream_t main = av1mi::ctx_stream(g->ctx);
  for (int p = 0; p < 3; p++) src[p] = dev_src ? dev_src[p] : s.d_in[p];
  if (!dev_src) {
    if (s.kernel_pending) G_HIP(hipStreamWaitEvent(g->up, s.filters_done, 0));
    if (s.kernel_pending && g->cfg.quality_stats) G_HIP(hipStreamWaitEvent(g->up, s.quality_done, 0));
    for (int p = 0; p < 3; p++)
      if (g->in_bytes[p]) G_HIP(hipMemcpyAsync(s.d_in[p], s.h_in[p], g->in_bytes[p], hipMemcpyHostToDevice, g->up));
    G_HIP(hipEventRecord(s.uploaded, g->up));
    s.upload_pending = true;
    G_HIP(hipStreamWaitEvent(main, s.uploaded, 0));
  }
  if (g->fmt != AV1MI_INPUT_PLANAR) {
    av1mi::InputLaunch L;
    memset(&L, 0, sizeof(L));
    for (int p = 0; p < 3; p++) { L.in[p] = src[p]; L.out[p] = g->scale ? s.d_pre[p] : s.d_src[p]; }
    L.ny = g->fed_ny; L.nc = g->fed_ny / 4;
    av1mi::ProfScope ps(g->ctx, AV1MI_K_INPUT, main);
    G_HIP(av1mi::launch_input_convert(g->fmt, L, main));
    for (int p = 0; p < 3; p++) src[p] = L.out[p];
  }
  if (g->chroma_stage) {
    const av1mi_gop_config &c = g->cfg;
    av1mi::ChromaLaunch L;
    for (int p = 0; p < 3; p++) { L.in[p] = src[p]; L.out[p] = g->scale ? s.d_pre[p] : s.d_src[p]; }
    L.chroma = c.source_chroma; L.src_bd = g->src_bd; L.bd = c.bit_depth; L.frames = c.segments;
    L.w = g->scale ? c.source_width : g->vw; L.h = g->scale ? c.source_height : g->vh;
    av1mi::ProfScope ps(g->ctx, AV1MI_K_INPUT, main);
    G_HIP(av1mi::launch_chroma_convert(L, main));
    for (int p = g->luma_through ? 1 : 0; p < 3; p++) src[p] = L.out[p];
  }
  if (g->scale) {
    av1mi::ProfScope ps(g->ctx, AV1MI_K_INPUT, main);
    G_HIP(av1mi::launch_scale(g->scale, g->cfg.segments, src, s.d_src, main));
    for (int p = 0; p < 3; p++) src[p] = s.d_src[p];
  }
  return AV1MI_OK;
}

static int code_blocks(av1mi_gop *g, Slot &s, int frame_type, const void *const src[3]) {
  const av1mi_gop_config &c = g->cfg;
  const int w = c.width, h = c.height;
  if (frame_type == 0) {
    av1mi_intra_job j;
    memset(&j, 0, sizeof(j));
    j.width = w; j.height = h; j.bit_depth = c.bit_depth; j.nframes = c.segments; j.qindex = s.q; j.block_size = 8; j.stride_y = g->plane[0].w; j.stride_uv = g->plane[1].w;
    j.d_src_y = src[0]; j.d_src_u = src[1]; j.d_src_v = src[2];
    j.d_rec_y = g->d_rec[0]; j.d_rec_u = g->d_rec[1]; j.d_rec_v = g->d_rec[2];
    j.d_lev_y = (int16_t *)s.d_lev[0]; j.d_lev_u = (int16_t *)s.d_lev[1]; j.d_lev_v = (int16_t *)s.d_lev[2];
    j.d_modes_y = (uint8_t *)s.d_modes[0]; j.d_modes_uv = (uint8_t *)s.d_modes[1];
    j.open_loop = g->intra_open_loop;
    if (!g->key32) {
      G_TRY(av1mi_intra_encode(g->ctx, &j));
    } else {
      const int hA = g->key_rows32, hB = h - hA;
      j.open_loop = 0; j.frame_rows = h; j.modes_frame_stride = g->key_modes_stride;
      if (hA) { j.height = hA; j.block_size = 32; G_TRY(av1mi_intra_encode(g->ctx, &j)); }
      if (hB) {
        size_t o[3];
        for (int p = 0; p < 3; p++) o[p] = (size_t)(hA >> g->plane[p].ss) * g->plane[p].w;
        j.height = hB; j.block_size = 8;
        j.d_src_y = (const char *)src[0] + o[0] * g->bps; j.d_src_u = (const char *)src[1] + o[1] * g->bps; j.d_src_v = (const char *)src[2] + o[2] * g->bps;
        j.d_rec_y = (char *)g->d_rec[0] + o[0] * g->bps; j.d_rec_u = (char *)g->d_rec[1] + o[1] * g->bps; j.d_rec_v = (char *)g->d_rec[2] + o[2] * g->bps;
        j.d_lev_y = (int16_t *)s.d_lev[0] + o[0]; j.d_lev_u = (int16_t *)s.d_lev[1] + o[1]; j.d_lev_v = (int16_t *)s.d_lev[2] + o[2];
        j.d_modes_y = (uint8_t *)s.d_modes[0] + g->key_modes_band; j.d_modes_uv = (uint8_t *)s.d_modes[1] + g->key_modes_band;
        G_TRY(av1mi_intra_encode(g->ctx, &j));
      }
    }
  } else {
    av1mi_inter_job j;
    memset(&j, 0, sizeof(j));
    j.width = w; j.height = h; j.bit_depth = c.bit_depth; j.nframes = c.segments; j.qindex = s.q; j.search_range = c.search_range; j.stride_y = g->plane[0].w; j.stride_uv = g->plane[1].w;
    j.d_src_y = src[0]; j.d_src_u = src[1]; j.d_src_v = src[2];
    j.d_ref_y = g->d_ref[0]; j.d_ref_u = g->d_ref[1]; j.d_ref_v = g->d_ref[2];
    j.d_rec_y = g->d_rec[0]; j.d_rec_u = g->d_rec[1]; j.d_rec_v = g->d_rec[2];
    j.d_lev_y = (int16_t *)s.d_lev[0]; j.d_lev_u = (int16_t *)s.d_lev[1]; j.d_lev_v = (int16_t *)s.d_lev[2];
    j.d_mvs = (int16_t *)s.d_mv; j.d_skip = (uint8_t *)s.d_skip;
    j.d_ref_alt_y = g->d_cdef[0]; j.d_ref_alt_u = g->d_cdef[1]; j.d_ref_alt_v = g->d_cdef[2];
    j.d_ref_sel = (const uint8_t *)g->slot[g->last].d_lr_on;
    j.coarse_range = c.coarse_range;
    G_TRY(av1mi::inter_encode_with(g->ctx, &j, g->d_me));
  }
  G_HIP(hipEventRecord(s.kernel_done, av1mi::ctx_stream(g->ctx)));
  s.kernel_pending = true;
  s.frame_type = frame_type;
  return AV1MI_OK;
}

static int download_symbols(av1mi_gop *g, Slot &s) {
  for (int p = 0; p < 3; p++) G_HIP(hipMemcpyAsync(s.h_lev[p], s.d_lev[p], g->plane[p].n * 2, hipMemcpyDeviceToHost, g->down));
  if (s.frame_type == 0) {
    for (int k = 0; k < 2; k++) G_HIP(hipMemcpyAsync(s.h_modes[k], s.d_modes[k], g->nb, hipMemcpyDeviceToHost, g->down));
  } else {
    G_HIP(hipMemcpyAsync(s.h_mv, s.d_mv, g->nb * 4, hipMemcpyDeviceToHost, g->down));
    G_HIP(hipMemcpyAsync(s.h_skip, s.d_skip, g->nb, hipMemcpyDeviceToHost, g->down));
  }
  return AV1MI_OK;
}

static int extend_plane(av1mi_gop *g, const Plane &P, void *d) {
  return av1mi_extend_frames(g->ctx, d, P.w, P.w, P.h, P.vw, P.vh, g->cfg.bit_depth, g->cfg.segments);
}

static int follow_q(av1mi_gop *g, const Slot &s) {
  const int t = s.frame_type, m = t == 0 && g->key32 ? 2 : t;
  const av1mi_frame_params &P = s.params;
  av1mi::LevelsLaunch L;
  memset(&L, 0, sizeof(L));
  if (g->mi_q[m] != s.q) {
    const size_t fy = (size_t)g->cfg.width * g->cfg.height;
    const uint32_t keep = ~0x00FFFF00u, hold = 1u << 24;
    L.a[L.arrays++] = { (uint32_t *)g->d_mi[m][0], fy / 16, keep, (uint32_t)P.lf_level[0] << 8 | (uint32_t)P.lf_level[1] << 16, hold };
    L.a[L.arrays++] = { (uint32_t *)g->d_mi[m][1], fy / 64, keep, (uint32_t)P.lf_level[2] << 8 | (uint32_t)P.lf_level[2] << 16, hold };
    g->mi_q[m] = s.q;
  }
  if (g->cdef_q[t] != s.q) {
    const size_t nsb = (size_t)((g->cfg.width + 63) / 64) * ((g->cfg.height + 63) / 64);
    L.a[L.arrays++] = { (uint32_t *)g->d_cdef_sb[t], nsb, 0u,
                        (uint32_t)(P.cdef_y >> 2) | (uint32_t)(P.cdef_y & 3) << 8 | (uint32_t)(P.cdef_uv >> 2) << 16 | (uint32_t)(P.cdef_uv & 3) << 24, 0u };
    g->cdef_q[t] = s.q;
  }
  if (!L.arrays) return AV1MI_OK;
  hipStream_t main = av1mi::ctx_stream(g->ctx);
  av1mi::ProfScope ps(g->ctx, AV1MI_K_MISC, main);
  G_HIP(av1mi::launch_mi_levels(L, main));
  return AV1MI_OK;
}

static int loop_filters(av1mi_gop *g, Slot &s, const void *const src[3]) {
  const av1mi_gop_config &c = g->cfg;
  const int w = c.width, h = c.height, S = c.segments, bd = c.bit_depth, key = s.frame_type == 0;
  const av1mi_frame_params &P = s.params;
  G_TRY(follow_q(g, s));
  for (int p = 0; p < 3; p++) {
    const Plane &L = g->plane[p];
    G_TRY(av1mi_deblock_frames(g->ctx, g->d_rec[p], L.w, g->d_dbl[p], L.w, L.w, L.h, bd, L.ss, (const uint32_t *)g->d_mi[key && g->key32 ? 2 : s.frame_type][L.ss], L.w / 4, 0,
                               P.lf_sharpness, S));
  }
  av1mi_cdef_job cj;
  memset(&cj, 0, sizeof(cj));
  cj.width = w; cj.height = h; cj.bit_depth = bd; cj.nframes = S; cj.damping = P.cdef_damping; cj.stride_y = g->plane[0].w; cj.stride_uv = g->plane[1].w;
  cj.d_src_y = g->d_dbl[0]; cj.d_src_u = g->d_dbl[1]; cj.d_src_v = g->d_dbl[2];
  cj.d_dst_y = g->d_cdef[0]; cj.d_dst_u = g->d_cdef[1]; cj.d_dst_v = g->d_cdef[2];
  cj.d_sb_strength = (const uint8_t *)g->d_cdef_sb[s.frame_type]; cj.sb_frame_stride = 0;
  cj.d_skip8 = (const uint8_t *)(key ? g->d_zero_skip : s.d_skip); cj.skip_frame_stride = key ? 0 : (size_t)(w / 8) * (h / 8);
  G_TRY(av1mi_cdef_frames(g->ctx, &cj));
  const bool padded = g->vw != w || g->vh != h;
  if (padded)
    for (int p = 0; p < 3; p++) { G_TRY(extend_plane(g, g->plane[p], g->d_dbl[p])); G_TRY(extend_plane(g, g->plane[p], g->d_cdef[p])); }
  av1mi_lr_decide_job lj;
  memset(&lj, 0, sizeof(lj));
  lj.width = w; lj.height = h; lj.bit_depth = bd; lj.nframes = S; lj.unit_size = P.lr_unit_size; lj.stride_y = g->plane[0].w; lj.stride_uv = g->plane[1].w;
  lj.d_cdef_y = g->d_cdef[0]; lj.d_cdef_u = g->d_cdef[1]; lj.d_cdef_v = g->d_cdef[2];
  lj.d_dbl_y = g->d_dbl[0]; lj.d_dbl_u = g->d_dbl[1]; lj.d_dbl_v = g->d_dbl[2];
  lj.d_out_y = g->d_ref[0]; lj.d_out_u = g->d_ref[1]; lj.d_out_v = g->d_ref[2];
  lj.d_orig_y = src[0]; lj.d_orig_u = src[1]; lj.d_orig_v = src[2];
  lj.d_units_y = (const int8_t *)g->d_lr[0]; lj.d_units_uv = (const int8_t *)g->d_lr[1];
  lj.d_scratch = g->d_lr_scratch; lj.d_on = (uint8_t *)s.d_lr_on;
  lj.no_self_guided_units = P.lr_unit_y[0] != 2 && P.lr_unit_uv[0] != 2;
  G_TRY(av1mi_lr_yuv_decide(g->ctx, &lj));
  if (padded)
    for (int p = 0; p < 3; p++) G_TRY(extend_plane(g, g->plane[p], g->d_ref[p]));
  G_HIP(hipEventRecord(s.filters_done, av1mi::ctx_stream(g->ctx)));
  if (s.symbols_down) {
    G_HIP(hipStreamWaitEvent(g->down, s.filters_done, 0));
    G_HIP(hipMemcpyAsync(s.h_lr_on, s.d_lr_on, (size_t)S * 3, hipMemcpyDeviceToHost, g->down));
    G_HIP(hipEventRecord(s.downloaded, g->down));
  }
  return AV1MI_OK;
}

static int measure_quality(av1mi_gop *g, Slot &s, const void *const src[3]) {
  hipStream_t main = av1mi::ctx_stream(g->ctx);
  av1mi::QualityLaunch Q;
  Q.bd = g->cfg.bit_depth; Q.w = g->vw; Q.h = g->vh; Q.frames = g->cfg.segments;
  Q.src = src; Q.dec0 = g->d_ref; Q.dec1 = g->d_cdef; Q.sel = (const uint8_t *)s.d_lr_on;
  Q.scratch = g->d_quality_scratch; Q.out = (av1mi_quality *)s.h_quality;
  {
    av1mi::ProfScope ps(g->ctx, AV1MI_K_QUALITY, main);
    G_HIP(av1mi::launch_quality(Q, main));
  }
  G_HIP(hipEventRecord(s.quality_done, main));
  return AV1MI_OK;
}

static int entropy_results(av1mi_gop *g, Slot &s, hipStream_t st) {
  const int S = g->cfg.segments;
  G_HIP(hipMemcpyAsync(s.h_tile_size, s.d_tile_size, (size_t)g->tiles * S * 4, hipMemcpyDeviceToHost, st));
  G_HIP(hipMemcpyAsync(s.h_total, s.d_total, 16, hipMemcpyDeviceToHost, st));
  G_HIP(hipMemcpyAsync(s.h_lr_on, s.d_lr_on, (size_t)S * 3, hipMemcpyDeviceToHost, st));
  G_HIP(hipEventRecord(s.ent_done, st));
  return AV1MI_OK;
}
static int finish_entropy(av1mi_gop *g, Slot &s, hipStream_t st) {
  G_TRY(av1mi::av1_entropy_back(g->ctx, s.ent_ticket, st));
  s.ent_ticket = -1;
  return entropy_results(g, s, st);
}

static int start_coder(av1mi_gop *g, Slot &s) {
  const av1mi_gop_config &c = g->cfg;
  const av1mi_frame_params &P = s.params;
  hipStream_t main = av1mi::ctx_stream(g->ctx), side = av1mi::ctx_side_stream(g->ctx), back = av1mi::ctx_back_stream(g->ctx);
  if (!side || !back) return av1mi::ctx_fail(g->ctx, AV1MI_E_DEVICE, "no side stream");
  if (g->coder_streams == 1) back = side;
  else if (g->coder_streams == 2) side = back = main;
  if (side != main) G_HIP(hipStreamWaitEvent(side, s.filters_done, 0));
  av1mi_av1_entropy_job ej;
  memset(&ej, 0, sizeof(ej));
  ej.width = c.width; ej.height = c.height; ej.nframes = c.segments; ej.key = s.frame_type == 0; ej.base_q_idx = s.q;
  ej.d_lev_y = (const int16_t *)s.d_lev[0]; ej.d_lev_u = (const int16_t *)s.d_lev[1]; ej.d_lev_v = (const int16_t *)s.d_lev[2];
  ej.d_modes_y = (const uint8_t *)s.d_modes[0]; ej.d_modes_uv = (const uint8_t *)s.d_modes[1];
  ej.d_mvs = (const int16_t *)s.d_mv; ej.d_skip = (const uint8_t *)s.d_skip;
  ej.lr_on[0] = P.lr_unit_y[0] == 1; ej.lr_on[1] = ej.lr_on[2] = P.lr_unit_uv[0] == 1;
  ej.d_lr_on = (const uint8_t *)s.d_lr_on;
  ej.visible_width = g->vw; ej.visible_height = g->vh;
  ej.key_rows32 = s.frame_type == 0 && g->key32 ? g->key_rows32 : 0;
  memcpy(ej.lr_unit_y, P.lr_unit_y, 8); memcpy(ej.lr_unit_uv, P.lr_unit_uv, 8);
  ej.d_out = (uint8_t *)s.h_ent_out; ej.out_cap = g->ent_cap; ej.d_tile_size = (uint32_t *)s.d_tile_size; ej.d_total = (uint64_t *)s.d_total;
  if (g->coder_streams == 3) {
    G_TRY(av1mi::av1_entropy_front(g->ctx, &ej, side, &s.ent_ticket));
    Slot &prev = g->slot[(g->submitted + kSlots - 1) % kSlots];
    if (g->submitted > 0 && prev.ent_ticket >= 0) G_TRY(finish_entropy(g, prev, main));
  } else {
    G_TRY(av1mi::av1_entropy_submit(g->ctx, &ej, side, back));
    G_TRY(entropy_results(g, s, back));
  }
  s.ent_pending = true;
  return AV1MI_OK;
}

static int submit_batch(av1mi_gop *g, int frame_type, const void *const *dev_src) {
  if (g->submitted - g->collected >= kSlots) return av1mi::ctx_fail(g->ctx, AV1MI_E_INVAL, "%d batches in flight: collect first", (int)kSlots);
  if (frame_type < -1 || frame_type > 1) return av1mi::ctx_fail(g->ctx, AV1MI_E_INVAL, "frame_type %d", frame_type);
  if (frame_type < 0) frame_type = g->gop_pos == 0 ? 0 : 1;
  if (frame_type == 1 && g->submitted == 0) return av1mi::ctx_fail(g->ctx, AV1MI_E_INVAL, "the first frame of a session must be a key frame");
  G_HIP(hipSetDevice(av1mi::ctx_device(g->ctx)));
  Slot &s = g->slot[g->submitted % kSlots];
  s.q = g->next_q;
  if (s.q == g->cfg.base_q_idx) s.params = g->params[frame_type];
  else frame_params(s.q, g->cfg.bit_depth, frame_type, &s.params);
  const void *src[3];
  G_TRY(feed_source(g, s, dev_src, src));
  if (s.ent_pending) G_HIP(hipStreamWaitEvent(av1mi::ctx_stream(g->ctx), s.ent_done, 0));
  G_TRY(code_blocks(g, s, frame_type, src));
  s.symbols_down = g->cfg.gpu_entropy != 1 || g->symbols_always;
  if (s.symbols_down) {
    G_HIP(hipStreamWaitEvent(g->down, s.kernel_done, 0));
    G_TRY(download_symbols(g, s));
  }
  G_TRY(loop_filters(g, s, src));
  if (g->cfg.quality_stats) G_TRY(measure_quality(g, s, src));
  if (g->cfg.gpu_entropy) G_TRY(start_coder(g, s));
  g->last = (int)(g->submitted % kSlots);
  g->submitted++;
  g->gop_pos = frame_type == 0 ? 1 % g->cfg.gop_length : (g->gop_pos + 1) % g->cfg.gop_length;
  g->acquired = false;
  return AV1MI_OK;
}

extern "C" {

int av1mi_gop_set_base_q_idx(av1mi_gop *g, int base_q_idx) {
  if (!g) return AV1MI_E_INVAL;
  if (base_q_idx < 1 || base_q_idx > 255) return av1mi::ctx_fail(g->ctx, AV1MI_E_INVAL, "base_q_idx %d must lie in 1..255", base_q_idx);
  g->next_q = base_q_idx;
  return AV1MI_OK;
}

int av1mi_gop_pending(av1mi_gop *g) { return g ? (int)(g->submitted - g->collected) : 0; }
long av1mi_gop_entropy_fallbacks(av1mi_gop *g) { return g ? g->fallbacks : 0; }

int av1mi_gop_acquire_input(av1mi_gop *g, void **y, void **u, void **v) {
  if (!g || !y || !u || !v) return AV1MI_E_INVAL;
  if (g->submitted - g->collected >= kSlots) return av1mi::ctx_fail(g->ctx, AV1MI_E_INVAL, "%d batches in flight: collect before acquiring the next input", (int)kSlots);
  G_HIP(hipSetDevice(av1mi::ctx_device(g->ctx)));
  Slot &s = g->slot[g->submitted % kSlots];
  if (s.upload_pending) { G_HIP(hipEventSynchronize(s.uploaded)); s.upload_pending = false; }
  *y = s.h_in[0]; *u = s.h_in[1]; *v = s.h_in[2];
  g->acquired = true;
  return AV1MI_OK;
}

int av1mi_gop_submit(av1mi_gop *g, int frame_type) {
  if (!g) return AV1MI_E_INVAL;
  if (!g->acquired) return av1mi::ctx_fail(g->ctx, AV1MI_E_INVAL, "submit without av1mi_gop_acquire_input");
  return submit_batch(g, frame_type, nullptr);
}

int av1mi_gop_submit_device(av1mi_gop *g, const void *d_y, const void *d_u, const void *d_v, int frame_type) {
  if (!g) return AV1MI_E_INVAL;
  if (g->fmt == AV1MI_INPUT_P010 || g->fmt == AV1MI_INPUT_NV12) d_v = d_u;
  if (g->chroma_stage && g->cfg.source_chroma == AV1MI_CHROMA_400) d_u = d_v = d_y;
  if (!d_y || !d_u || !d_v || (((uintptr_t)d_y | (uintptr_t)d_u | (uintptr_t)d_v) & (g->fmt == AV1MI_INPUT_PLANAR && !g->chroma_stage ? 7 : 15)))
    return av1mi::ctx_fail(g->ctx, AV1MI_E_INVAL, "null or misaligned device source plane");
  const void *src[3] = { d_y, d_u, d_v };
  return submit_batch(g, frame_type, src);
}

int av1mi_gop_collect(av1mi_gop *g, av1mi_gop_frame *out) {
  if (!g || !out) return AV1MI_E_INVAL;
  if (g->submitted == g->collected) return av1mi::ctx_fail(g->ctx, AV1MI_E_INVAL, "nothing in flight");
  G_HIP(hipSetDevice(av1mi::ctx_device(g->ctx)));
  Slot &s = g->slot[g->collected % kSlots];
  if (s.symbols_down) G_HIP(hipEventSynchronize(s.downloaded));
  memset(out, 0, sizeof(*out));
  out->params = s.params;
  out->lr_on = (const uint8_t *)s.h_lr_on;
  if (g->cfg.quality_stats) { G_HIP(hipEventSynchronize(s.quality_done)); out->quality = (const av1mi_quality *)s.h_quality; }
  out->segments = g->cfg.segments;
  out->blocks_per_frame = g->nb / (size_t)g->cfg.segments;
  out->key_block_size = s.frame_type == 0 && g->key32 ? 32 : 8;
  out->key_modes_stride = g->key_modes_stride; out->key_modes_band = g->key_modes_band;
  auto symbols = [&](bool levels) {
    if (s.frame_type == 0) { out->y_mode = (const uint8_t *)s.h_modes[0]; out->uv_mode = (const uint8_t *)s.h_modes[1]; }
    else { out->mv = (const int16_t *)s.h_mv; out->skip = (const uint8_t *)s.h_skip; }
    if (levels) { out->lev_y = (const int16_t *)s.h_lev[0]; out->lev_u = (const int16_t *)s.h_lev[1]; out->lev_v = (const int16_t *)s.h_lev[2]; }
  };
  if (s.symbols_down) symbols(true);
  if (g->cfg.gpu_entropy) {
    if (s.ent_ticket >= 0) G_TRY(finish_entropy(g, s, av1mi::ctx_stream(g->ctx)));
    G_HIP(hipEventSynchronize(s.ent_done));
    const uint64_t total = ((const uint64_t *)s.h_total)[0], status = ((const uint64_t *)s.h_total)[1];
    if (status || total > g->ent_cap) {
      if (getenv("AV1MI_DEBUG"))
        fprintf(stderr, "[av1mi] batch %ld (frame type %d) falls back to the host coder: status %llx (1 list / records, 2 payload slot, 4 output), %llu bytes of %zu\n",
                (long)g->collected, s.frame_type, (unsigned long long)status, (unsigned long long)total, g->ent_cap);
      if (!s.symbols_down) {
        for (Slot &o : g->slot)
          for (int p = 0; p < 3; p++)
            if (!o.h_lev[p]) G_TRY(host_alloc(g, &o.h_lev[p], g->plane[p].n * 2));
        G_TRY(download_symbols(g, s));
        G_HIP(hipStreamSynchronize(g->down));
        symbols(true);
      }
      if (g->fallbacks + 1 >= kFallbacksToHostMode) g->symbols_always = true;
      g->fallbacks++;
    } else {
      out->tiles_per_frame = g->tiles; out->tile_size = (const uint32_t *)s.h_tile_size; out->tile_payload = (const uint8_t *)s.h_ent_out; out->payload_bytes = total;
    }
  }
  g->collected++;
  return AV1MI_OK;
}

int av1mi_gop_download_reference(av1mi_gop *g, void *y, void *u, void *v) {
  if (!g || !y || !u || !v) return AV1MI_E_INVAL;
  G_TRY(av1mi_sync(g->ctx));
  const int S = g->cfg.segments;
  std::vector<uint8_t> on((size_t)S * 3, 1);
  if (g->submitted) G_TRY(av1mi_download(g->ctx, on.data(), g->slot[g->last].d_lr_on, on.size()));
  void *dst[3] = { y, u, v };
  for (int p = 0; p < 3; p++) {
    const size_t per = g->plane[p].bytes / (size_t)S;
    for (int sg = 0; sg < S; sg++)
      G_TRY(av1mi_download(g->ctx, (char *)dst[p] + per * sg, (const char *)(on[(size_t)sg * 3 + p] ? g->d_ref[p] : g->d_cdef[p]) + per * sg, per));
  }
  return AV1MI_OK;
}

}
```

### av1-go_amd/host/av1_bitstream.hpp

```cpp
#pragma once
#include <cstddef>
#include <cstdint>
#include <string>
#include <vector>

#include "../../include/av1mi_host.h"

namespace av1mi_host {
namespace av1 {

struct SequenceParams {
  int width = 0, height = 0, bit_depth = 8;
  bool operator==(const SequenceParams &o) const { return width == o.width && height == o.height && bit_depth == o.bit_depth; }
};

inline int visible_width(const av1mi_obu_frame &f) { return f.visible_width ? f.visible_width : f.width; }
inline int visible_height(const av1mi_obu_frame &f) { return f.visible_height ? f.visible_height : f.height; }
inline SequenceParams sequence_params(const av1mi_obu_frame &f) {
  SequenceParams sp; sp.width = visible_width(f); sp.height = visible_height(f); sp.bit_depth = f.bit_depth;
  return sp;
}
std::vector<uint8_t> temporal_delimiter_obu();
std::vector<uint8_t> sequence_header_obu(const SequenceParams &sp);
bool frame_obu(const av1mi_obu_frame &f, int threads, std::vector<uint8_t> *out, std::string *err);
bool frame_obu_from_tiles(const av1mi_obu_frame &f, const uint8_t *payloads, const uint32_t *sizes, int ntiles, std::vector<uint8_t> *out,
                          std::string *err);
std::vector<uint8_t> range_code_raw(const uint32_t *fl, const uint32_t *fh, const uint8_t *sym, const uint8_t *nsym, size_t count);
bool opstream_supported(const av1mi_obu_frame &f, std::string *why);
bool opstream_tiles(const av1mi_obu_frame &f, std::vector<std::vector<uint8_t>> *tiles, std::string *err, int key_rows32 = 0);
int opstream_slots();
int opstream_tile32(const av1mi_obu_frame &f, int sbr, int sbc, uint32_t ops_cap, uint32_t *list, uint32_t *grouped, uint16_t *slot_total, uint16_t *slot_base,
                    std::string *err);
bool blocks_temporal_unit(const av1mi_obu_blocks &d, bool with_sequence_header, std::vector<uint8_t> *out, std::string *err, int threads = 1,
                          const size_t (*tile_start)[2] = nullptr);
bool temporal_unit(const av1mi_obu_frame &f, bool with_sequence_header, int threads, std::vector<uint8_t> *out, std::string *err);

}
}
```

### av1-go_amd/host/av1_opstream.cpp

```cpp
#include <algorithm>
#include <cstdio>
#include <cstdlib>
#include <cstring>
#include <string>
#include <vector>
#include "../csrc/av1_ops_cdfs.hpp"
#include "av1_bitstream.hpp"

namespace av1mi_host {
namespace av1 {

bool opstream_supported(const av1mi_obu_frame &f, std::string *why) {
  auto no = [&](const char *m) { if (why) *why = m; return false; };
  if (f.cdef_bits || f.reduced_tx_set || f.disable_cdf_update) return no("cdef_bits / reduced_tx_set / disable_cdf_update must be 0");
  if (f.tile_cols_log2 >= 0 || f.tile_rows_log2 >= 0) return no("one superblock per tile only");
  if (f.angle_y || f.angle_uv || f.cfl_alpha || f.tx_type || f.is_inter) return no("angle deltas, chroma from luma, transform types and intra blocks in inter frames are host-writer only");
  if (f.frame_type == 0 && f.skip) return no("key frames are coded with skip = 0");
  for (int p = 0; p < 3; p++) if (f.lr_type[p] > 1) return no("Wiener restoration only");
  if (f.lr_unit_shift || f.lr_uv_shift) return no("64x64 restoration units only");
  return true;
}

namespace {
bool code_list(std::vector<av1ops::op_t> &list, const std::vector<uint32_t> &grouped, int nslots, const uint16_t *total, const uint16_t *base,
               const av1ops::SlotTable &tab, const uint16_t *image, std::vector<uint8_t> *out, std::string *err) {
  using namespace av1ops;
  const int nops = (int)list.size();
  for (int sl = 0; sl < nslots; sl++)
    if (total[sl]) run_chain(&image[tab.off[sl]], tab.nsym[sl], &grouped[(size_t)base[sl]], total[sl], list.data());
  out->resize((size_t)nops * 2 + 64);
  Coder c;
  uint16_t stage[Coder::kStage];
  c.init(out->data(), (int)out->size(), stage);
  for (int i = 0; i < nops; i++) code_word(c, list[(size_t)i]);
  const int n = c.finish();
  if (n < 0) { if (err) *err = "tile payload overflow"; return false; }
  out->resize((size_t)n);
  return true;
}
template <int kBlocks>
bool code_tile(const uint16_t *rec, int block_records, const int *nrec, const int *first, uint16_t *pos, int nslots, const uint16_t *total,
               const uint16_t *base, int run, const av1ops::SlotTable &tab, const uint16_t *image, std::vector<uint8_t> *out, std::string *err) {
  using namespace av1ops;
  if (run > 65535) { if (err) *err = "tile too large for 16-bit entry positions"; return false; }
  std::vector<op_t> list((size_t)first[kBlocks], 0);
  std::vector<uint32_t> grouped((size_t)run, 0);
  for (int b = 0; b < kBlocks; b++) replay_block<kBlocks>(rec + (size_t)b * block_records, nrec[b], pos, b, first[b], list.data(), grouped.data());
  return code_list(list, grouped, nslots, total, base, tab, image, out, err);
}
struct WaveLoop {
  template <class T> using Var = av1ops::LaneVar<T, av1ops::kLanes32>;
  template <class F> void each(F f) { for (int lane = 0; lane < av1ops::kLanes32; lane++) f(lane); }
  int scan(Var<int> &v) {
    int run = 0;
    for (int lane = 0; lane < av1ops::kLanes32; lane++) { const int x = v.v[lane]; v.v[lane] = run; run += x; }
    return run;
  }
  int first(Var<int> &v) { return v.v[0]; }
};
void frame_view_of(const av1mi_obu_frame &f, av1ops::FrameView *v) {
  memset(v, 0, sizeof(*v));
  v->w8 = f.width / 8; v->h8 = f.height / 8; v->key = f.frame_type == 0;
  v->y_mode = f.y_mode; v->uv_mode = f.uv_mode; v->mv = f.mv; v->skip = f.skip; v->lev_y = f.lev_y; v->lev_u = f.lev_u; v->lev_v = f.lev_v;
  for (int p = 0; p < 3; p++) {
    v->lr_on[p] = f.lr_type[p] == 1;
    const int ph = p ? (visible_height(f) + 1) >> 1 : visible_height(f), pw = p ? (visible_width(f) + 1) >> 1 : visible_width(f);
    v->lr_rows[p] = std::max((ph + 32) / 64, 1); v->lr_cols[p] = std::max((pw + 32) / 64, 1);
  }
}
bool lr_units_of(const av1mi_obu_frame &f, av1ops::FrameView *v, std::string *err) {
  for (int p = 0; p < 3; p++) {
    if (!v->lr_on[p]) continue;
    const int8_t *u = f.lr_units[p];
    const size_t n = (size_t)v->lr_rows[p] * v->lr_cols[p];
    for (size_t i = 1; i < n; i++) if (memcmp(u, u + i * 8, 8)) { if (err) *err = "restoration units must be uniform per plane"; return false; }
    if (p == 2 && v->lr_on[1] && memcmp(u, f.lr_units[1], 8)) { if (err) *err = "U and V restoration units must be equal"; return false; }
    memcpy(v->lr_unit[p ? 1 : 0], u, 8);
  }
  return true;
}
}

bool opstream_tiles(const av1mi_obu_frame &f, std::vector<std::vector<uint8_t>> *tiles, std::string *err, int key_rows32) {
  using namespace av1ops;
  if (!opstream_supported(f, err)) return false;
  if (key_rows32 && (f.frame_type != 0 || (key_rows32 & 63) || key_rows32 > f.height || (f.width & 31))) { if (err) *err = "bad 32x32 band"; return false; }
  FrameView v;
  frame_view_of(f, &v);
  std::vector<uint8_t> zskip;
  if (!v.key && !v.skip) { zskip.assign((size_t)v.w8 * v.h8, 0); v.skip = zskip.data(); }
  if (!lr_units_of(f, &v, err)) return false;
  const size_t nb = (size_t)v.w8 * v.h8;
  std::vector<BlockInfo> info(nb);
  v.info = info.data();
  for (size_t b = 0; b < nb; b++) { memset(&info[b], 0, sizeof(BlockInfo)); block_summary(v, (int)b, &info[b]); }
  if (!v.key) for (int r = 0; r < v.h8; r++) for (int c = 0; c < v.w8; c++) inter_mode_decision(v, r, c, &info[(size_t)r * v.w8 + c]);
  const int qcat = q_category(f.base_q_idx);
  SlotTable tab;
  const std::vector<uint16_t> image = default_slot_image(v.key != 0, qcat, &tab);
  const int sbr_n = (v.h8 + 7) / 8, sbc_n = (v.w8 + 7) / 8;
  tiles->assign((size_t)sbr_n * sbc_n, {});
  const int nslots = v.key ? S_KEY_END : S_INTER_END;
  std::vector<uint8_t> cnt((size_t)S_MAX * kBlocksPerTile);
  std::vector<uint16_t> pos((size_t)S_MAX * kBlocksPerTile), rec((size_t)kBlocksPerTile * kBlockRecords);
  ScanTables scan;
  fill_scan_tables(&scan);
  alignas(16) uint8_t mag[kMagBytes];
  const TokScratch ts = { mag, &scan };
  const bool stats = getenv("AV1MI_TOK_STATS") != nullptr;
  int st_rec = 0, st_cnt = 0, st_ops = 0, st_over = 0; long st_ops_sum = 0;
  SlotTable tab32;
  const std::vector<uint16_t> image32 = key_rows32 ? default_slot_image_k32(qcat, &tab32) : std::vector<uint16_t>();
  std::vector<Tile32Mem> mem32(key_rows32 ? 1 : 0);
  const uint32_t ops_cap32 = 1u << 20;
  std::vector<op_t> list32(key_rows32 ? ops_cap32 : 0);
  std::vector<uint32_t> grouped32(key_rows32 ? 65536 : 0);
  for (int sbr = 0; sbr < sbr_n; sbr++)
    for (int sbc = 0; sbc < sbc_n; sbc++) {
      if (sbr * 64 < key_rows32) {
        WaveLoop wave;
        uint16_t base[S_MAX], total[S_MAX];
        const int words = tok_tile32(wave, mem32[0], v, sbr, sbc, list32.data(), ops_cap32, grouped32.data(), total, base);
        if (words < 0) { if (err) *err = "tile too large for 16-bit entry positions"; return false; }
        std::vector<op_t> list(list32.begin(), list32.begin() + words);
        if (!code_list(list, grouped32, K_END, total, base, tab32, image32.data(), &(*tiles)[(size_t)sbr * sbc_n + sbc], err)) return false;
        continue;
      }
      std::fill(cnt.begin(), cnt.end(), 0);
      int first[kBlocksPerTile + 1], nrec[kBlocksPerTile];
      first[0] = 0;
      bool over = false;
      for (int zi = 0; zi < kBlocksPerTile; zi++) {
        Sink k = { &rec[(size_t)zi * kBlockRecords], cnt.data(), zi, 0, 0, false };
        tok_block(v, k, ts, sbr, sbc, zi);
        if (k.overflow && !stats) { if (err) *err = "a block exceeds the tokenizer's record area"; return false; }
        over |= k.overflow;
        nrec[zi] = k.nrec;
        first[zi + 1] = first[zi] + k.n;
        if (k.nrec > st_rec) st_rec = k.nrec;
      }
      if (stats) {
        for (uint8_t c : cnt) if (c > st_cnt) st_cnt = c;
        if (first[kBlocksPerTile] > st_ops) st_ops = first[kBlocksPerTile];
        st_ops_sum += first[kBlocksPerTile];
        if (over) { st_over++; continue; }
      }
      uint16_t base[S_MAX], total[S_MAX];
      int run = 0;
      for (int sl = 0; sl < nslots; sl++) {
        const int n = group_positions(&cnt[(size_t)sl * kBlocksPerTile], &pos[(size_t)sl * kBlocksPerTile], run);
        base[sl] = (uint16_t)run; total[sl] = (uint16_t)n;
        run = (run + n + kListAlign - 1) & ~(kListAlign - 1);
      }
      if (!code_tile<kBlocksPerTile>(rec.data(), kBlockRecords, nrec, first, pos.data(), nslots, total, base, run, tab, image.data(),
                                     &(*tiles)[(size_t)sbr * sbc_n + sbc], err))
        return false;
    }
  if (stats)
    fprintf(stderr, "[av1mi tok stats] %d tiles: records per block <= %d (capacity %d), symbols of a slot in a block <= %d (255), list words per tile <= %d, mean %.0f; %d tiles over a block capacity\n",
            sbr_n * sbc_n, st_rec, (int)kBlockRecords, st_cnt, st_ops, (double)st_ops_sum / (sbr_n * sbc_n), st_over);
  return true;
}

int opstream_slots() { return av1ops::S_MAX; }

int opstream_tile32(const av1mi_obu_frame &f, int sbr, int sbc, uint32_t ops_cap, uint32_t *list, uint32_t *grouped, uint16_t *slot_total, uint16_t *slot_base,
                    std::string *err) {
  using namespace av1ops;
  if (!opstream_supported(f, err) || f.frame_type != 0 || (f.width & 31) || sbr < 0 || sbc < 0 || (sbr + 1) * 64 > f.height || sbc * 64 >= f.width) return -2;
  FrameView v;
  frame_view_of(f, &v);
  if (!lr_units_of(f, &v, err)) return -2;
  std::vector<Tile32Mem> mem(1);
  WaveLoop wave;
  return tok_tile32(wave, mem[0], v, sbr, sbc, list, ops_cap, grouped, slot_total, slot_base);
}

}
}
```

### av1-go_amd/host/capi_host.cpp

```cpp
#include <cstring>
#include "daemon.hpp"
#include "av1_bitstream.hpp"
#include "mux.hpp"
#include "y4m.hpp"
#include "backend.hpp"
#include "../csrc/quality.hpp"

using namespace av1mi_host;

extern "C" {
int av1mi_host_determine_quality(int height) { return DetermineQuality(height); }
int av1mi_host_check_size_gate(long long orig, long long neu, double ratio) { return CheckSizeGate(orig, neu, ratio) ? 1 : 0; }
int av1mi_host_transcode_args(const char *in, const char *out, int has_video, int index, int height, int webrip, char *buf, int cap) {
  ProbeResult pr; pr.has_video_stream = has_video != 0; pr.VideoStream.Index = index; pr.VideoStream.Height = height;
  std::vector<std::string> a; std::string err;
  const bool ok = TranscodeArgs("ffmpeg", in, out, pr, webrip != 0, &a, &err);
  std::string j;
  if (ok) for (size_t i = 0; i < a.size(); i++) j += (i ? "\n" : "") + a[i]; else j = err;
  strncpy(buf, j.c_str(), cap - 1); buf[cap - 1] = 0;
  return ok ? (int)a.size() : -1;
}
int av1mi_host_job_args(const char *in, const char *out, int height, int webrip, double target_bpp, char *buf, int cap) {
  ProbeResult pr; pr.has_video_stream = true; pr.VideoStream.Height = height;
  std::vector<std::string> a; std::string err;
  if (!TranscodeArgs("ffmpeg", in, out, pr, webrip != 0, &a, &err)) return -1;
  TranscodeConfig cfg; cfg.TargetBitsPerPixel = target_bpp;
  AppendConfigArgs(cfg, &a);
  std::string j;
  for (size_t i = 0; i < a.size(); i++) j += (i ? "\n" : "") + a[i];
  strncpy(buf, j.c_str(), cap - 1); buf[cap - 1] = 0;
  return (int)a.size();
}
int av1mi_host_parse_rate_options(const char *joined, long long *out, char *err, int cap) {
  std::vector<std::string> a; std::string s = joined; size_t p = 0, q;
  while ((q = s.find('\n', p)) != std::string::npos) { a.push_back(s.substr(p, q - p)); p = q + 1; }
  a.push_back(s.substr(p));
  BackendJob job; std::string e;
  const bool ok = ParseBackendJob(a, &job, &e);
  strncpy(err, e.c_str(), cap - 1); err[cap - 1] = 0;
  out[0] = job.bitrate; out[1] = job.target_bpp_u; out[2] = job.qmin; out[3] = job.qmax; out[4] = job.quality;
  return ok ? 0 : -1;
}
long long av1mi_host_y4m_scan(const char *path, int group, unsigned long long *sum, int *seekable, int *geometry, char *err, int cap) {
  Y4mSource y;
  std::string e;
  auto fail = [&]() { strncpy(err, e.c_str(), cap - 1); err[cap - 1] = 0; return -1LL; };
  if (!y.open(path, &e)) return fail();
  const int cw = (y.w + 7) & ~7, ch = (y.h + 7) & ~7;
  const size_t bps = y.bd == 8 ? 1 : 2;
  std::vector<unsigned char> Y((size_t)cw * ch * bps), U((size_t)cw * ch * bps / 4), V((size_t)cw * ch * bps / 4);
  unsigned long long acc = 1469598103934665603ull;
  long long total = 0;
  for (long first = 0;; first += group) {
    const long n = y.prepare(first, group, &e);
    if (n < 0) return fail();
    if (n == 0) break;
    for (long i = 0; i < n; i++) {
      if (!y.read(i, cw, ch, Y.data(), U.data(), V.data())) { e = "read failed"; return fail(); }
      for (const auto *pl : { &Y, &U, &V }) for (unsigned char b : *pl) acc = (acc ^ b) * 1099511628211ull;
    }
    total += n;
  }
  *sum = acc; *seekable = y.seekable() ? 1 : 0;
  geometry[0] = y.w; geometry[1] = y.h; geometry[2] = y.bd; geometry[3] = y.fps_n; geometry[4] = y.fps_d;
  return total;
}
int av1mi_host_y4m_layout(const char *path, int any_layout, int *geometry, unsigned long long *frame_bytes, long long *frames, char *err, int cap) {
  Y4mSource y;
  std::string e;
  if (!y.open(path, &e, any_layout != 0)) { strncpy(err, e.c_str(), cap - 1); err[cap - 1] = 0; return -1; }
  geometry[0] = y.w; geometry[1] = y.h; geometry[2] = y.bd; geometry[3] = y.chroma; geometry[4] = y.src_bd;
  *frame_bytes = y.frame_bytes(); *frames = y.known_frames();
  return 0;
}
int av1mi_host_parse_format_option(const char *joined, char *err, int cap) {
  std::vector<std::string> a; std::string s = joined; size_t p = 0, q;
  while ((q = s.find('\n', p)) != std::string::npos) { a.push_back(s.substr(p, q - p)); p = q + 1; }
  a.push_back(s.substr(p));
  BackendJob job; std::string e;
  const bool ok = ParseBackendJob(a, &job, &e);
  strncpy(err, e.c_str(), cap - 1); err[cap - 1] = 0;
  return ok ? (job.to_420 ? 1 : 0) : -1;
}
int av1mi_host_y4m_sar(const char *path, int *sar) {
  Y4mSource y;
  std::string e;
  if (!y.open(path, &e)) return -1;
  sar[0] = y.sar_n; sar[1] = y.sar_d;
  return 0;
}
int av1mi_host_scale_target(int iw, int ih, int sar_n, int sar_d, const char *chain, int *w, int *h) {
  std::string e;
  bool square = false;
  return ScaleTarget(iw, ih, sar_n, sar_d, chain ? chain : "", w, h, &square, &e) ? 0 : -1;
}
int av1mi_host_mux_selftest(const char *out_path, int width, int height, int bit_depth, int fps_n, int fps_d, const unsigned char *units,
                            const long long *off, int n_units, int gop, const char *sides, char *err, int cap) {
  std::string e;
  auto fail = [&]() { strncpy(err, e.c_str(), cap - 1); err[cap - 1] = 0; return -1; };
  StreamSink sink;
  for (std::string rest = sides ? sides : ""; !rest.empty();) {
    const size_t nl = rest.find('\n');
    const std::string one = rest.substr(0, nl);
    rest = nl == std::string::npos ? "" : rest.substr(nl + 1);
    if (!one.empty() && !sink.add_side_file(one, &e)) return fail();
  }
  av1::SequenceParams sp;
  sp.width = width; sp.height = height; sp.bit_depth = bit_depth;
  if (!sink.open(out_path, sp, fps_n, fps_d, &e)) return fail();
  for (int i = 0; i < n_units; i++) {
    const std::vector<uint8_t> tu(units + off[i], units + off[i + 1]);
    if (!sink.write(tu, i % gop == 0, &e)) { sink.abort(); return fail(); }
  }
  if (!sink.close(&e)) return fail();
  return 0;
}
int av1mi_run_transcode(int argc, const char *const *argv, char *err, size_t errcap) {
  std::vector<std::string> a;
  for (int i = 0; i < argc; i++) a.push_back(argv[i] ? argv[i] : "");
  const RunResult rr = RunTranscode("av1mi", a);
  if (err && errcap) { strncpy(err, rr.err.c_str(), errcap - 1); err[errcap - 1] = 0; }
  return rr.exitCode;
}
int av1mi_host_run_transcode(const char *joined, char *buf, int cap) {
  std::vector<std::string> a; std::string s = joined; size_t p = 0, q;
  while ((q = s.find('\n', p)) != std::string::npos) { a.push_back(s.substr(p, q - p)); p = q + 1; }
  a.push_back(s.substr(p));
  const RunResult rr = RunTranscode("av1mi", a);
  strncpy(buf, rr.err.c_str(), cap - 1); buf[cap - 1] = 0;
  return rr.exitCode;
}
int av1mi_host_process_job(const char *source, long long orig_size, double ratio, const char *state_dir, int wait_s, int replace_source,
                           char *status, char *reason, int cap) {
  Job job; job.ID = "test"; job.SourcePath = source; job.OriginalSize = orig_size;
  TranscodeConfig cfg; cfg.MaxSizeRatio = ratio; cfg.JobStateDir = state_dir ? state_dir : ""; cfg.StableWaitSeconds = wait_s;
  cfg.ReplaceSource = replace_source != 0;
  ProbeResult pr; pr.HasVideo = true; pr.has_video_stream = true; pr.VideoStream.Height = 720;
  const std::string e = ProcessJob(&job, "av1mi", pr, cfg);
  strncpy(status, job.Status.c_str(), cap - 1); status[cap - 1] = 0;
  strncpy(reason, job.Reason.c_str(), cap - 1); reason[cap - 1] = 0;
  return e.empty() ? 0 : 1;
}
int av1mi_host_process_job_q(const char *source, long long orig_size, double ratio, const char *state_dir, int wait_s, int replace_source,
                             char *status, char *reason, int cap, double min_psnr) {
  Job job; job.ID = "test"; job.SourcePath = source; job.OriginalSize = orig_size;
  TranscodeConfig cfg; cfg.MaxSizeRatio = ratio; cfg.JobStateDir = state_dir ? state_dir : ""; cfg.StableWaitSeconds = wait_s;
  cfg.ReplaceSource = replace_source != 0; cfg.MinPSNR = min_psnr;
  ProbeResult pr; pr.HasVideo = true; pr.has_video_stream = true; pr.VideoStream.Height = 720;
  const std::string e = ProcessJob(&job, "av1mi", pr, cfg);
  strncpy(status, job.Status.c_str(), cap - 1); status[cap - 1] = 0;
  strncpy(reason, job.Reason.c_str(), cap - 1); reason[cap - 1] = 0;
  return e.empty() ? 0 : 1;
}
int av1mi_quality_planes_host(int bit_depth, int width, int height, int frames, const void *const src[3], const void *const dec0[3], const void *const dec1[3],
                              const uint8_t *select, av1mi_quality *out) {
  return av1mi::quality::planes_host(bit_depth, width, height, frames, src, dec0, dec1, select, out);
}
double av1mi_quality_psnr(const av1mi_quality *q, int bit_depth) { return av1mi::quality::psnr_from_sse((double)q->sse, (double)q->samples, bit_depth); }
double av1mi_quality_ssim(const av1mi_quality *q) { return q->ssim_sum / (double)q->windows; }
void av1mi_host_quality_constants(int bit_depth, long long *c1, long long *c2) { *c1 = av1mi::quality::ssim_c1(bit_depth); *c2 = av1mi::quality::ssim_c2(bit_depth); }
int av1mi_host_parse_quality_options(const char *joined, char *stats_path, int cap, double *min_psnr, char *err, int errcap) {
  std::vector<std::string> a; std::string s = joined; size_t p = 0, q;
  while ((q = s.find('\n', p)) != std::string::npos) { a.push_back(s.substr(p, q - p)); p = q + 1; }
  a.push_back(s.substr(p));
  BackendJob job; std::string e;
  const bool ok = ParseBackendJob(a, &job, &e);
  strncpy(stats_path, job.stats_path.c_str(), cap - 1); stats_path[cap - 1] = 0;
  strncpy(err, e.c_str(), errcap - 1); err[errcap - 1] = 0;
  *min_psnr = job.min_psnr;
  return ok ? 0 : -1;
}
int av1mi_host_quality_summary_line(const av1mi_quality *q, const long long *bytes, int n, int bit_depth, char *buf, int cap) {
  av1mi::quality::Summary sum;
  long long total = 0;
  for (int i = 0; i < n; i++) { sum.add(q + 3 * i, bit_depth); total += bytes[i]; }
  int k = snprintf(buf, cap, "summary frames:%ld bytes:%lld", sum.frames, total);
  if (k < 0 || k >= cap) return -1;
  return k + av1mi::quality::format_figures(sum.figures(bit_depth), buf + k, (size_t)(cap - k));
}
long long av1mi_obu_write_temporal_unit(const av1mi_obu_frame *f, int with_sequence_header, int threads, uint8_t *out, long long cap,
                                        char *err, int errcap) {
  std::vector<uint8_t> b; std::string e;
  if (!av1::temporal_unit(*f, with_sequence_header != 0, threads, &b, &e)) {
    if (err && errcap > 0) { strncpy(err, e.c_str(), errcap - 1); err[errcap - 1] = 0; }
    return -1;
  }
  if ((long long)b.size() <= cap && out) memcpy(out, b.data(), b.size());
  return (long long)b.size();
}
long long av1mi_session_temporal_unit(const av1mi_gop_frame *fr, int seg, int width, int height, int bit_depth, int visible_width, int visible_height,
                                      int with_sequence_header, int threads, uint8_t *out, long long cap, char *err, int errcap) {
  std::vector<uint8_t> b; std::string e;
  if (!fr || seg < 0 || seg >= fr->segments) e = "bad batch / segment";
  else if (SessionTemporalUnit(*fr, seg, width, height, bit_depth, visible_width, visible_height, with_sequence_header != 0, threads, &b, &e)) {
    if ((long long)b.size() <= cap && out) memcpy(out, b.data(), b.size());
    return (long long)b.size();
  }
  if (err && errcap > 0) { strncpy(err, e.c_str(), errcap - 1); err[errcap - 1] = 0; }
  return -1;
}
long long av1mi_obu_write_blocks_temporal_unit(const av1mi_obu_blocks *f, int with_sequence_header, uint8_t *out, long long cap, char *err, int errcap) {
  std::vector<uint8_t> b; std::string e;
  if (!f || !av1::blocks_temporal_unit(*f, with_sequence_header != 0, &b, &e)) {
    if (err && errcap > 0) { strncpy(err, f ? e.c_str() : "null description", errcap - 1); err[errcap - 1] = 0; }
    return -1;
  }
  if ((long long)b.size() <= cap && out) memcpy(out, b.data(), b.size());
  return (long long)b.size();
}
long long av1mi_obu_assemble_temporal_unit(const av1mi_obu_frame *f, const uint8_t *payloads, const uint32_t *sizes, int ntiles,
                                           int with_sequence_header, uint8_t *out, long long cap, char *err, int errcap) {
  std::vector<uint8_t> fr; std::string e;
  if (!av1::frame_obu_from_tiles(*f, payloads, sizes, ntiles, &fr, &e)) {
    if (err && errcap > 0) { strncpy(err, e.c_str(), errcap - 1); err[errcap - 1] = 0; }
    return -1;
  }
  std::vector<uint8_t> b = av1::temporal_delimiter_obu();
  if (with_sequence_header) {
    const av1::SequenceParams sp = av1::sequence_params(*f);
    const std::vector<uint8_t> sh = av1::sequence_header_obu(sp);
    b.insert(b.end(), sh.begin(), sh.end());
  }
  b.insert(b.end(), fr.begin(), fr.end());
  if ((long long)b.size() <= cap && out) memcpy(out, b.data(), b.size());
  return (long long)b.size();
}
long long av1mi_host_opstream_key32_temporal_unit(const av1mi_obu_frame *f, int key_rows32, int with_sequence_header, uint8_t *out, long long cap, char *err,
                                                  int errcap) {
  std::vector<std::vector<uint8_t>> tiles; std::string e;
  auto fail = [&](long long code) { if (err && errcap > 0) { strncpy(err, e.c_str(), errcap - 1); err[errcap - 1] = 0; } return code; };
  if (!av1::opstream_supported(*f, &e)) return fail(-2);
  if (!av1::opstream_tiles(*f, &tiles, &e, key_rows32)) return fail(-1);
  std::vector<uint8_t> cat; std::vector<uint32_t> sizes;
  for (auto &t : tiles) { sizes.push_back((uint32_t)t.size()); cat.insert(cat.end(), t.begin(), t.end()); }
  std::vector<uint8_t> fr;
  if (!av1::frame_obu_from_tiles(*f, cat.data(), sizes.data(), (int)sizes.size(), &fr, &e)) return fail(-1);
  std::vector<uint8_t> b = av1::temporal_delimiter_obu();
  if (with_sequence_header) {
    const av1::SequenceParams sp = av1::sequence_params(*f);
    const std::vector<uint8_t> sh = av1::sequence_header_obu(sp);
    b.insert(b.end(), sh.begin(), sh.end());
  }
  b.insert(b.end(), fr.begin(), fr.end());
  if ((long long)b.size() <= cap && out) memcpy(out, b.data(), b.size());
  return (long long)b.size();
}
int av1mi_host_opstream_slots(void) { return av1::opstream_slots(); }
int av1mi_host_opstream_tile32(const av1mi_obu_frame *f, int sbr, int sbc, uint32_t ops_cap, uint32_t *list, uint32_t *grouped, uint16_t *slot_total,
                               uint16_t *slot_base) {
  if (!f || !list || !grouped || !slot_total || !slot_base) return -2;
  std::string e;
  return av1::opstream_tile32(*f, sbr, sbc, ops_cap, list, grouped, slot_total, slot_base, &e);
}
long long av1mi_host_opstream_temporal_unit(const av1mi_obu_frame *f, int with_sequence_header, uint8_t *out, long long cap, char *err, int errcap) {
  return av1mi_host_opstream_key32_temporal_unit(f, 0, with_sequence_header, out, cap, err, errcap);
}
int av1mi_host_job_json(const char *id, const char *source, const char *status, const char *reason, long long orig, long long neu, char *buf, int cap) {
  Job j; j.ID = id; j.SourcePath = source; j.Status = status; j.Reason = reason; j.OriginalSize = orig; j.NewSize = neu; j.CreatedAt = "2026-01-02T03:04:05Z";
  const std::string s = JobToJSON(j);
  strncpy(buf, s.c_str(), cap - 1); buf[cap - 1] = 0;
  return (int)s.size();
}
double av1mi_host_gpu_usage(int device, const char *sysfs_root) { return GetGPUUsage(device, sysfs_root ? sysfs_root : "/sys"); }
int av1mi_host_mux_units(const char *path, int w, int h, int bd, int fps_n, int fps_d, const uint8_t *data, const long long *sizes,
                         const uint8_t *keys, int n) {
  StreamSink sink; std::string err;
  av1::SequenceParams sp; sp.width = w; sp.height = h; sp.bit_depth = bd;
  if (!sink.open(path, sp, fps_n, fps_d, &err)) return 1;
  for (int i = 0; i < n; i++) {
    std::vector<uint8_t> tu(data, data + sizes[i]);
    data += sizes[i];
    if (!sink.write(tu, keys[i] != 0, &err)) { sink.abort(); return 2; }
  }
  return sink.close(&err) ? 0 : 3;
}
int av1mi_host_mux_units_display(const char *path, int w, int h, int bd, int fps_n, int fps_d, const uint8_t *data, const long long *sizes,
                                 const uint8_t *keys, int n, int display_w, int display_h) {
  StreamSink sink; std::string err;
  av1::SequenceParams sp; sp.width = w; sp.height = h; sp.bit_depth = bd;
  if (display_w || display_h) sink.set_display_size(display_w, display_h);
  if (!sink.open(path, sp, fps_n, fps_d, &err)) return 1;
  for (int i = 0; i < n; i++) {
    std::vector<uint8_t> tu(data, data + sizes[i]);
    data += sizes[i];
    if (!sink.write(tu, keys[i] != 0, &err)) { sink.abort(); return 2; }
  }
  return sink.close(&err) ? 0 : 3;
}
int av1mi_host_job_pool(const char *sources, int workers, int ngpus, double ratio, const char *state_dir, char *buf, int cap) {
  std::vector<Job> jobs; std::string s = sources; size_t p = 0, q;
  auto add = [&](const std::string &path) {
    Job j; j.ID = "pool" + std::to_string(jobs.size()); j.SourcePath = path;
    FILE *f = fopen(path.c_str(), "rb");
    if (f) { fseek(f, 0, SEEK_END); j.OriginalSize = ftell(f); fclose(f); }
    jobs.push_back(j);
  };
  while ((q = s.find('\n', p)) != std::string::npos) { add(s.substr(p, q - p)); p = q + 1; }
  add(s.substr(p));
  TranscodeConfig cfg; cfg.MaxSizeRatio = ratio; cfg.JobStateDir = state_dir ? state_dir : ""; cfg.StableWaitSeconds = 0;
  ProbeResult pr; pr.HasVideo = true; pr.has_video_stream = true; pr.VideoStream.Height = 720;
  std::vector<std::string> errs;
  const PoolStats ps = RunJobPool(&jobs, workers, ngpus, pr, cfg, &errs);
  std::string out;
  for (size_t i = 0; i < jobs.size(); i++) out += (i ? "\n" : "") + jobs[i].Status + (errs[i].empty() ? "" : ": " + errs[i]);
  strncpy(buf, out.c_str(), cap - 1); buf[cap - 1] = 0;
  return ps.succeeded;
}
}
```

Before: 2901.

## Fold block summaries into 8x8 tile tokenizer and skip info kernel on key frames

Measured after the change: 2979, median of 6. 2.7% higher.

```diff
diff --git a/av1-go_amd/csrc/av1_entropy_kernels.hip b/av1-go_amd/csrc/av1_entropy_kernels.hip
--- a/av1-go_amd/csrc/av1_entropy_kernels.hip
+++ b/av1-go_amd/csrc/av1_entropy_kernels.hip
@@ -1,7 +1,7 @@
 #include <string.h>
 #include <vector>
 #include "av1_ops_cdfs.hpp"
-#include "av1_ops32.hpp"
+#include "av1_ops8.hpp"
 #include "av1mi_internal.hpp"
 
 namespace av1mi {
@@ -43,117 +43,13 @@
   const long nb = (long)L.fv.w8 * L.fv.h8, i = (long)blockIdx.x * 256 + threadIdx.x;
   if (i >= nb * L.nframes) return;
   const int f = (int)(i / nb), b = (int)(i - (long)f * nb);
-  const FrameView v = frame_view(L, f);
+  const FrameView v = frame_view<0>(L, f);
   BlockInfo o = {};
-  block_summary(v, b, &o);
-  if (!v.key) inter_mode_decision(v, b / v.w8, b % v.w8, &o);
+  inter_mode_decision(v, b / v.w8, b % v.w8, &o);
   L.info[nb * f + b] = o;
 }
 
-constexpr int kReplaySlots = (S_MAX + 1) / 2;
-struct TokLds {
-  union {
-    struct { uint8_t cnt[S_MAX * kBlocksPerTile]; alignas(16) uint8_t mag[kBlocksPerTile * kMagBytes]; } p1;
-    uint16_t pos[kReplaySlots * kBlocksPerTile];
-  };
-  uint16_t total[S_MAX], base[S_MAX];
-  ScanTables scan;
-};
-
-__global__ __launch_bounds__(64) __attribute__((amdgpu_waves_per_eu(2, 8))) void k_av1_tokens(Av1EntLaunch L) {
-  const int tiles = L.sbr_n * L.sbc_n, t = blockIdx.x, f = t / tiles, tt = t - f * tiles, sbr = tt / L.sbc_n, sbc = tt - sbr * L.sbc_n;
-  if (sbr < L.sb_rows32) return;
-  const FrameView v = frame_view(L, f);
-  const int zi = threadIdx.x, nslots = v.key ? S_KEY_END : S_INTER_END;
-  __shared__ TokLds S;
-  {
-    uint32_t *m = reinterpret_cast<uint32_t *>(S.p1.cnt);
-    for (int i = zi; i < S_MAX * kBlocksPerTile / 4; i += 64) m[i] = 0;
-    if (zi == 0) fill_scan_tables(&S.scan);
-  }
-  __syncthreads();
-  const int below = tiles - L.sb_rows32 * L.sbc_n;
-  uint16_t *rec = L.rec + (((size_t)f * below + (tt - (tiles - below))) * kBlocksPerTile + zi) * kBlockRecords;
-  const TokScratch ts = { S.p1.mag + zi * kMagBytes, &S.scan };
-  Sink k = { rec, S.p1.cnt, zi, 0, 0, false };
-  tok_block(v, k, ts, sbr, sbc, zi);
-  int x = k.n;
-#pragma unroll
-  for (int d = 1; d < 64; d <<= 1) {
-    const int y = __shfl_up(x, d, 64);
-    if (zi >= d) x += y;
-  }
-  const int total = __shfl(x, 63, 64), first = x - k.n;
-  if ((uint32_t)total > L.ops_cap || __any(k.overflow)) {
-    if (zi == 0) { atomicOr(L.status, 1u); L.nops[t] = 0; }
-    for (int sl = zi; sl < S_MAX; sl += 64) L.slot_total[(size_t)t * S_MAX + sl] = 0;
-    return;
-  }
-  if (zi == 0) L.nops[t] = (uint32_t)total;
-  __syncthreads();
-  constexpr int kOwn = (S_MAX + 63) / 64;
-  uint32_t c[kOwn][kBlocksPerTile / 4];
-#pragma unroll
-  for (int q = 0; q < kOwn; q++) {
-    const int sl = zi + 64 * q;
-    int sum = 0;
-#pragma unroll
-    for (int w = 0; w < kBlocksPerTile / 4; w++) {
-      const uint32_t u = sl < nslots ? reinterpret_cast<const uint32_t *>(S.p1.cnt)[sl * (kBlocksPerTile / 4) + w] : 0u;
-      c[q][w] = u;
-      sum = (int)__builtin_amdgcn_sad_u8(u, 0u, (unsigned)sum);
-    }
-    if (sl < S_MAX) S.total[sl] = (uint16_t)sum;
-  }
-  __syncthreads();
-  {
-    int mine = 0;
-    for (int q = 0; q < 4; q++) { const int sl = 4 * zi + q; if (sl < nslots) mine += (S.total[sl] + kListAlign - 1) & ~(kListAlign - 1); }
-    int inc = mine;
-#pragma unroll
-    for (int d = 1; d < 64; d <<= 1) {
-      const int y = __shfl_up(inc, d, 64);
-      if (zi >= d) inc += y;
-    }
-    int run = inc - mine;
-    for (int q = 0; q < 4; q++) { const int sl = 4 * zi + q; if (sl < nslots) { S.base[sl] = (uint16_t)run; run += (S.total[sl] + kListAlign - 1) & ~(kListAlign - 1); } }
-  }
-  __syncthreads();
-#pragma unroll
-  for (int q = 0; q < kOwn; q++) {
-    const int sl = zi + 64 * q;
-    if (sl >= S_MAX) continue;
-    const bool on = sl < nslots;
-    L.slot_total[(size_t)t * S_MAX + sl] = on ? S.total[sl] : (uint16_t)0;
-    L.slot_base[(size_t)t * S_MAX + sl] = on ? S.base[sl] : (uint16_t)0;
-  }
-  op_t *list = L.ops + (size_t)t * L.ops_cap;
-  uint32_t *grouped = L.grouped + (size_t)t * L.grouped_cap;
-#pragma unroll
-  for (int half = 0; half < 2; half++) {
-    const int lo = half * kReplaySlots, hi = lo + kReplaySlots;
-    if (half) __syncthreads();
-#pragma unroll
-    for (int q = 0; q < kOwn; q++) {
-      const int sl = zi + 64 * q;
-      if (sl < lo || sl >= hi || sl >= nslots) continue;
-      int run = S.base[sl];
-#pragma unroll
-      for (int w = 0; w < kBlocksPerTile / 4; w++) {
-        const uint32_t u = c[q][w];
-        const int p0 = run, p1 = p0 + (int)(u & 0xFF), p2 = p1 + (int)((u >> 8) & 0xFF), p3 = p2 + (int)((u >> 16) & 0xFF);
-        run = p3 + (int)(u >> 24);
-        uint32_t *d = reinterpret_cast<uint32_t *>(S.pos + (sl - lo) * kBlocksPerTile + 4 * w);
-        d[0] = (uint32_t)p0 | ((uint32_t)p1 << 16); d[1] = (uint32_t)p2 | ((uint32_t)p3 << 16);
-      }
-    }
-    __syncthreads();
-    __threadfence_block();
-    replay_block<kBlocksPerTile>(rec, k.nrec, S.pos, zi, first, list, grouped, lo, hi, half == 0);
-  }
-}
-
-struct Wave32 {
+struct TileWave {
   template <class T> using Var = LaneVar<T, 1>;
   template <class F> __device__ __forceinline__ void each(F f) { f((int)threadIdx.x); __syncthreads(); }
   __device__ __forceinline__ int scan(Var<int> &v) {
@@ -169,12 +65,29 @@
   }
   __device__ __forceinline__ int first(Var<int> &v) { return __shfl(v.v[0], 0, 64); }
 };
+
+__global__ __launch_bounds__(64) __attribute__((amdgpu_waves_per_eu(2, 8))) void k_av1_tokens(Av1EntLaunch L) {
+  const int tiles = L.sbr_n * L.sbc_n, t = blockIdx.x, f = t / tiles, tt = t - f * tiles, sbr = tt / L.sbc_n, sbc = tt - sbr * L.sbc_n;
+  if (sbr < L.sb_rows32) return;
+  const FrameView v = frame_view(L, f);
+  __shared__ Tile8Mem S;
+  const int below = tiles - L.sb_rows32 * L.sbc_n;
+  uint16_t *rec = L.rec + ((size_t)f * below + (tt - (tiles - below))) * kBlocksPerTile * kBlockRecords;
+  TileWave w;
+  const int n = tok_tile8(w, S, v, sbr, sbc, rec, L.ops + (size_t)t * L.ops_cap, L.ops_cap, L.grouped + (size_t)t * L.grouped_cap,
+                          L.slot_total + (size_t)t * S_MAX, L.slot_base + (size_t)t * S_MAX);
+  if (threadIdx.x == 0) {
+    if (n < 0) atomicOr(L.status, 1u);
+    L.nops[t] = n < 0 ? 0u : (uint32_t)n;
+  }
+}
+
 __global__ __launch_bounds__(64) void k_av1_tokens32(Av1EntLaunch L) {
   __shared__ Tile32Mem S;
   const int tiles = L.sbr_n * L.sbc_n, band = L.sb_rows32 * L.sbc_n, f = blockIdx.x / band, tt = blockIdx.x - f * band, sbr = tt / L.sbc_n, sbc = tt - sbr * L.sbc_n;
   const size_t t = (size_t)f * tiles + tt;
   const FrameView v = frame_view<1>(L, f);
-  Wave32 w;
+  TileWave w;
   const int n = tok_tile32(w, S, v, sbr, sbc, L.ops + t * L.ops_cap, L.ops_cap, L.grouped + t * L.grouped_cap, L.slot_total + t * S_MAX, L.slot_base + t * S_MAX);
   if (threadIdx.x == 0) {
     if (n < 0) atomicOr(L.status, 1u);
@@ -336,7 +249,7 @@
   const long nb = (long)L.fv.w8 * L.fv.h8 * L.nframes;
   const int ntiles_all = L.sbr_n * L.sbc_n * L.nframes, ngroups = (ntiles_all + 63) / 64;
   ProfToken t = ctx_prof_begin(ctx, AV1MI_K_ENTROPY_TOKENS, s);
-  hipLaunchKernelGGL(k_av1_info, dim3((unsigned)((nb + 255) / 256)), dim3(256), 0, s, L);
+  if (!L.fv.key) hipLaunchKernelGGL(k_av1_info, dim3((unsigned)((nb + 255) / 256)), dim3(256), 0, s, L);
   if (L.sb_rows32 < L.sbr_n) hipLaunchKernelGGL(k_av1_tokens, dim3((unsigned)ntiles_all), dim3(64), 0, s, L);
   if (L.sb_rows32) hipLaunchKernelGGL(k_av1_tokens32, dim3((unsigned)(L.sb_rows32 * L.sbc_n * L.nframes)), dim3(64), 0, s, L);
   ctx_prof_end(ctx, t, s);
diff --git a/av1-go_amd/csrc/av1_ops.hpp b/av1-go_amd/csrc/av1_ops.hpp
--- a/av1-go_amd/csrc/av1_ops.hpp
+++ b/av1-go_amd/csrc/av1_ops.hpp
@@ -119,31 +119,7 @@
     if (nbits > 0) put(0x8000u | ((unsigned)nbits << 11) | (v & ((1u << nbits) - 1u)));
   }
 };
-AV1_HD int group_positions(const uint8_t *cnt_slot, uint16_t *pos_slot, int base) {
-  int run = base;
-  for (int b = 0; b < kBlocksPerTile; b++) { const int c = cnt_slot[b]; pos_slot[b] = (uint16_t)run; run += c; }
-  return run - base;
-}
-template <int kBlocks>
-AV1_HD void replay_block(const uint16_t *rec, int nrec, uint16_t *pos, int blk, int first, op_t *list, uint32_t *grouped, int slot_lo = 0,
-                         int slot_hi = 1 << 16, bool literals = true) {
-  int n = first;
-  for (int i0 = 0; i0 < nrec; i0 += 8) {
-    struct alignas(16) R8 { uint32_t w[4]; } q = *reinterpret_cast<const R8 *>(rec + i0);
-    AV1_UNROLL
-    for (int j = 0; j < 8; j++, n++) {
-      if (i0 + j >= nrec) break;
-      const unsigned r = (q.w[j >> 1] >> (16 * (j & 1))) & 0xFFFFu;
-      if (r & 0x8000u) { if (literals) list[n] = op_lit((int)((r >> 11) & 15), r & 0x7FFu); }
-      else {
-        const int sl = (int)(r >> 4);
-        if (sl >= slot_lo && sl < slot_hi) { uint16_t &p = pos[(sl - slot_lo) * kBlocks + blk]; grouped[p] = ((uint32_t)n << 4) | (r & 15u); p++; }
-      }
-    }
-  }
-}
-
-struct BlockInfo { uint8_t cul[3], dc[3], mode, flags; uint8_t num, drl; int16_t px, py; uint8_t pad[2]; };
+struct BlockInfo { uint8_t mode, flags, num, drl; int16_t px, py; };
 struct FrameView {
   int w8, h8;
   int key;
@@ -172,17 +148,20 @@
   *bx = x; *by = y;
 }
 
-AV1_HD void block_summary(const FrameView &f, int b, BlockInfo *o) {
-  const int16_t *p[3] = { f.lev_y + (long)b * 64, f.lev_u + (long)b * 16, f.lev_v + (long)b * 16 };
-  const bool skip = !f.key && f.skip[b];
-  for (int pl = 0; pl < 3; pl++) {
-    int cul = 0;
-    const int n = pl ? 16 : 64;
-    for (int i = 0; i < n; i++) cul += iabs(p[pl][i]);
-    o->cul[pl] = skip ? 0 : (uint8_t)imin(cul, 63);
-    o->dc[pl] = skip ? 0 : (uint8_t)(p[pl][0] < 0 ? 1 : p[pl][0] > 0 ? 2 : 0);
-  }
-}
+AV1_HD unsigned block_levels_summary(const FrameView &f, int b) {
+  if (!f.key && f.skip[b]) return 0;
+  auto cls = [](int v) { return v < 0 ? 1u : v > 0 ? 2u : 0u; };
+  unsigned s = cls(f.lev_y[(long)b * 64]);
+  for (int p = 1; p < 3; p++) {
+    const int16_t *lev = (p == 1 ? f.lev_u : f.lev_v) + (long)b * 16;
+    struct alignas(16) L8 { uint32_t w[4]; } q0 = *reinterpret_cast<const L8 *>(lev), q1 = *reinterpret_cast<const L8 *>(lev + 8);
+    const uint32_t any = q0.w[0] | q0.w[1] | q0.w[2] | q0.w[3] | q1.w[0] | q1.w[1] | q1.w[2] | q1.w[3];
+    s |= cls(lev[0]) << (2 * p) | (any ? 64u << (p - 1) : 0u);
+  }
+  return s;
+}
+AV1_HD int summary_dc(unsigned s, int p) { return (int)((s >> (2 * p)) & 3u); }
+AV1_HD int summary_cul(unsigned s, int p) { return p ? (int)((s >> (5 + p)) & 1u) : 0; }
 
 struct MvCand { int16_t x, y; int weight; };
 struct MvStack { MvCand st[8]; int num, new_ctx, ref_ctx; };
@@ -473,7 +452,7 @@
   }
 }
 
-AV1_HD void tok_block(const FrameView &f, Sink &k, const TokScratch &ts, int sbr, int sbc, int zi) {
+AV1_HD void tok_block(const FrameView &f, Sink &k, const TokScratch &ts, int sbr, int sbc, int zi, const uint8_t *sums) {
   int bx, by;
   demorton8((unsigned)zi, &bx, &by);
   const int r8 = sbr * 8 + by, c8 = sbc * 8 + bx;
@@ -482,8 +461,7 @@
   tok_partition_prefix(f, k, sbr, sbc, bx, by);
   const int b = r8 * f.w8 + c8;
   const bool au = by > 0, al = bx > 0;
-  const BlockInfo zero = {};
-  const BlockInfo ia = au ? f.info[b - f.w8] : zero, il = al ? f.info[b - 1] : zero;
+  const unsigned sa = au ? sums[(by - 1) * 8 + bx] : 0u, sl = al ? sums[by * 8 + bx - 1] : 0u;
   const int skip = f.key ? 0 : f.skip[b];
   k.sym(S_SKIP + (au && !f.key ? f.skip[b - f.w8] : 0) + (al && !f.key ? f.skip[b - 1] : 0), skip);
   int ym = 0;
@@ -500,7 +478,7 @@
     const int mode = me.mode & 3, ref_idx = me.mode >> 2, num = me.num;
     const int mx = f.mv[2 * b], my = f.mv[2 * b + 1];
     const int close = (au ? 1 : 0) + (al ? 1 : 0);
-    int num_new = (au ? ia.flags & 1 : 0) + (al ? il.flags & 1 : 0);
+    int num_new = (au ? f.info[b - f.w8].flags & 1 : 0) + (al ? f.info[b - 1].flags & 1 : 0);
     if (au && bx < 7 && c8 + 1 < f.w8 && morton8((unsigned)bx + 1, (unsigned)by - 1) < morton8((unsigned)bx, (unsigned)by)) num_new += f.info[b - f.w8 + 1].flags & 1;
     const int new_ctx = close == 0 ? 0 : close == 1 ? 3 - imin(num_new, 1) : 5 - imin(num_new, 1);
     const int ref_ctx = close == 0 ? 0 : close == 1 ? 3 : 5;
@@ -532,10 +510,10 @@
     }
   }
   if (skip) return;
-  tok_coeffs<8, kSlots8>(k, ts, false, f.lev_y + (long)b * 64, ia.cul[0], ia.dc[0], il.cul[0], il.dc[0], f.key ? S_INTRA_TX + ym : S_INTER_TX, f.key ? 1 : 7);
+  tok_coeffs<8, kSlots8>(k, ts, false, f.lev_y + (long)b * 64, 0, summary_dc(sa, 0), 0, summary_dc(sl, 0), f.key ? S_INTRA_TX + ym : S_INTER_TX, f.key ? 1 : 7);
   AV1_NOUNROLL
   for (int p = 1; p < 3; p++)
-    tok_coeffs<4, kSlots8>(k, ts, true, (p == 1 ? f.lev_u : f.lev_v) + (long)b * 16, ia.cul[p], ia.dc[p], il.cul[p], il.dc[p], -1, 0);
+    tok_coeffs<4, kSlots8>(k, ts, true, (p == 1 ? f.lev_u : f.lev_v) + (long)b * 16, summary_cul(sa, p), summary_dc(sa, p), summary_cul(sl, p), summary_dc(sl, p), -1, 0);
 }
 
 template <class F> AV1_HD void build_slot_table(int n, F nsym, SlotTable *t) {
diff --git a/av1-go_amd/csrc/av1_ops8.hpp b/av1-go_amd/csrc/av1_ops8.hpp
--- /dev/null
+++ b/av1-go_amd/csrc/av1_ops8.hpp
@@ -0,0 +1,138 @@
+#pragma once
+#include "av1_ops32.hpp"
+
+namespace av1ops {
+
+enum { kLanes8 = kBlocksPerTile, kReplaySlots = (S_MAX + 1) / 2, kOwn8 = (S_MAX + kLanes8 - 1) / kLanes8 };
+static_assert(2 * kReplaySlots >= S_MAX && S_MAX <= 256 && kOwn8 * kLanes8 >= S_MAX && 4 * kLanes8 >= S_MAX, "rows are bytes; two passes cover every slot");
+
+struct Tile8Mem {
+  union {
+    struct { uint8_t cnt[S_MAX * kBlocksPerTile]; alignas(16) uint8_t mag[kBlocksPerTile * kMagBytes]; } p1;
+    uint16_t pos[kReplaySlots * kBlocksPerTile];
+  };
+  uint16_t total[S_MAX], base[S_MAX];
+  uint8_t row[(S_MAX + 3) & ~3];
+  uint8_t sums[kBlocksPerTile];
+  ScanTables scan;
+};
+struct SlotCounts8 { uint32_t w[kOwn8][kBlocksPerTile / 4]; };
+
+AV1_HD void replay_block8(const uint16_t *rec, int nrec, uint16_t *pos, const uint8_t *row, int blk, int first, op_t *list, uint32_t *grouped, int row_lo,
+                          bool literals) {
+  int n = first;
+  for (int i0 = 0; i0 < nrec; i0 += 8) {
+    struct alignas(16) R8 { uint32_t w[4]; } q = *reinterpret_cast<const R8 *>(rec + i0);
+    AV1_UNROLL
+    for (int j = 0; j < 8; j++, n++) {
+      if (i0 + j >= nrec) break;
+      const unsigned r = (q.w[j >> 1] >> (16 * (j & 1))) & 0xFFFFu;
+      if (r & 0x8000u) { if (literals) list[n] = op_lit((int)((r >> 11) & 15), r & 0x7FFu); }
+      else {
+        const unsigned rw = (unsigned)row[r >> 4] - (unsigned)row_lo;
+        if (rw < (unsigned)kReplaySlots) { uint16_t &p = pos[rw * kBlocksPerTile + blk]; grouped[p] = ((uint32_t)n << 4) | (r & 15u); p++; }
+      }
+    }
+  }
+}
+
+template <class W>
+AV1_HD int tok_tile8(W &w, Tile8Mem &S, const FrameView &f, int sbr, int sbc, uint16_t *rec, op_t *list, uint32_t ops_cap, uint32_t *grouped,
+                     uint16_t *slot_total, uint16_t *slot_base) {
+  typedef typename W::template Var<int> LaneInt;
+  const int nslots = f.key ? S_KEY_END : S_INTER_END;
+  w.each([&](int lane) {
+    for (int i = lane; i < S_MAX * kBlocksPerTile / 4; i += kLanes8) reinterpret_cast<u32a *>(S.p1.cnt)[i] = 0;
+    if (lane == 0) fill_scan_tables(&S.scan);
+    int bx, by;
+    demorton8((unsigned)lane, &bx, &by);
+    const int r8 = sbr * 8 + by, c8 = sbc * 8 + bx;
+    S.sums[by * 8 + bx] = (uint8_t)(r8 < f.h8 && c8 < f.w8 ? block_levels_summary(f, r8 * f.w8 + c8) : 0u);
+  });
+  LaneInt nrec, first;
+  w.each([&](int lane) {
+    const TokScratch ts = { S.p1.mag + lane * kMagBytes, &S.scan };
+    Sink k = { rec + (size_t)lane * kBlockRecords, S.p1.cnt, lane, 0, 0, false };
+    tok_block(f, k, ts, sbr, sbc, lane, S.sums);
+    nrec[lane] = k.nrec;
+    first[lane] = k.n | (k.overflow ? 1 << 24 : 0);
+  });
+  const int sum = w.scan(first), words = sum & 0xFFFFFF;
+  bool fits = (uint32_t)words <= ops_cap && !(sum >> 24);
+  typename W::template Var<SlotCounts8> cnt;
+  if (fits) w.each([&](int lane) {
+    SlotCounts8 &c = cnt[lane];
+    AV1_UNROLL
+    for (int q = 0; q < kOwn8; q++) {
+      const int sl = lane + kLanes8 * q;
+      int tot = 0;
+      AV1_UNROLL
+      for (int i = 0; i < kBlocksPerTile / 4; i++) {
+        const uint32_t u = sl < nslots ? reinterpret_cast<const u32a *>(S.p1.cnt)[sl * (kBlocksPerTile / 4) + i] : 0u;
+        c.w[q][i] = u;
+#if defined(__HIP_DEVICE_COMPILE__)
+        tot = (int)__builtin_amdgcn_sad_u8(u, 0u, (unsigned)tot);
+#else
+        tot += (int)((u & 0xFF) + ((u >> 8) & 0xFF) + ((u >> 16) & 0xFF) + (u >> 24));
+#endif
+      }
+      if (sl < S_MAX) S.total[sl] = (uint16_t)tot;
+    }
+  });
+  LaneInt ent, used;
+  if (fits) w.each([&](int lane) {
+    int e = 0, u = 0;
+    for (int q = 0; q < 4; q++) {
+      const int sl = 4 * lane + q;
+      if (sl < nslots) { e += (S.total[sl] + kListAlign - 1) & ~(kListAlign - 1); u += S.total[sl] != 0; }
+    }
+    ent[lane] = e; used[lane] = u;
+  });
+  const int entries = fits ? w.scan(ent) : 0, rows = fits ? w.scan(used) : 0;
+  fits = fits && entries <= 65535;
+  if (!fits) {
+    w.each([&](int lane) { for (int sl = lane; sl < S_MAX; sl += kLanes8) slot_total[sl] = 0; });
+    return -1;
+  }
+  w.each([&](int lane) {
+    int run = ent[lane], r = used[lane];
+    for (int q = 0; q < 4; q++) {
+      const int sl = 4 * lane + q;
+      if (sl >= nslots) break;
+      const int tot = S.total[sl];
+      S.base[sl] = (uint16_t)run; S.row[sl] = (uint8_t)r;
+      run += (tot + kListAlign - 1) & ~(kListAlign - 1); r += tot != 0;
+    }
+  });
+  const int npass = rows <= kReplaySlots ? 1 : 2;
+  for (int pass = 0; pass < npass; pass++) {
+    const int row_lo = pass * kReplaySlots;
+    w.each([&](int lane) {
+      const SlotCounts8 &c = cnt[lane];
+      AV1_UNROLL
+      for (int q = 0; q < kOwn8; q++) {
+        const int sl = lane + kLanes8 * q;
+        if (sl >= S_MAX) continue;
+        if (pass == 0) { const bool on = sl < nslots; slot_total[sl] = on ? S.total[sl] : (uint16_t)0; slot_base[sl] = on ? S.base[sl] : (uint16_t)0; }
+        if (sl >= nslots || !S.total[sl]) continue;
+        const unsigned rw = (unsigned)S.row[sl] - (unsigned)row_lo;
+        if (rw >= (unsigned)kReplaySlots) continue;
+        int run = S.base[sl];
+        AV1_UNROLL
+        for (int i = 0; i < kBlocksPerTile / 4; i++) {
+          const uint32_t u = c.w[q][i];
+          const int p0 = run, p1 = p0 + (int)(u & 0xFF), p2 = p1 + (int)((u >> 8) & 0xFF), p3 = p2 + (int)((u >> 16) & 0xFF);
+          run = p3 + (int)(u >> 24);
+          u32a *d = reinterpret_cast<u32a *>(S.pos + rw * kBlocksPerTile + 4 * i);
+          d[0] = (uint32_t)p0 | ((uint32_t)p1 << 16); d[1] = (uint32_t)p2 | ((uint32_t)p3 << 16);
+        }
+      }
+    });
+    w.each([&](int lane) {
+      replay_block8(rec + (size_t)lane * kBlockRecords, nrec[lane], S.pos, S.row, lane, first[lane] & 0xFFFFFF, list, grouped, row_lo, pass == 0);
+    });
+  }
+  return words;
+}
+
+}
diff --git a/av1-go_amd/csrc/gop_session.hip b/av1-go_amd/csrc/gop_session.hip
--- a/av1-go_amd/csrc/gop_session.hip
+++ b/av1-go_amd/csrc/gop_session.hip
@@ -281,7 +281,7 @@
   }
   if (c.gpu_entropy) {
     g->tiles = ((w + 63) / 64) * ((h + 63) / 64);
-    g->ent_cap = (size_t)w * h * S;
+    g->ent_cap = (size_t)w * h * S * 3 * c.bit_depth / 16;
   }
   G_HIP(hipSetDevice(av1mi::ctx_device(g->ctx)));
   if (c.source_width) G_HIP(av1mi::scale_plan_create(c.bit_depth, c.source_width, c.source_height, g->vw, g->vh, &g->scale));
diff --git a/av1-go_amd/host/av1_bitstream.hpp b/av1-go_amd/host/av1_bitstream.hpp
--- a/av1-go_amd/host/av1_bitstream.hpp
+++ b/av1-go_amd/host/av1_bitstream.hpp
@@ -31,6 +31,8 @@
 int opstream_slots();
 int opstream_tile32(const av1mi_obu_frame &f, int sbr, int sbc, uint32_t ops_cap, uint32_t *list, uint32_t *grouped, uint16_t *slot_total, uint16_t *slot_base,
                     std::string *err);
+int opstream_tile8(const av1mi_obu_frame &f, int sbr, int sbc, uint32_t ops_cap, uint32_t *list, uint32_t *grouped, uint16_t *slot_total, uint16_t *slot_base,
+                   std::string *err);
 bool blocks_temporal_unit(const av1mi_obu_blocks &d, bool with_sequence_header, std::vector<uint8_t> *out, std::string *err, int threads = 1,
                           const size_t (*tile_start)[2] = nullptr);
 bool temporal_unit(const av1mi_obu_frame &f, bool with_sequence_header, int threads, std::vector<uint8_t> *out, std::string *err);
diff --git a/av1-go_amd/host/av1_opstream.cpp b/av1-go_amd/host/av1_opstream.cpp
--- a/av1-go_amd/host/av1_opstream.cpp
+++ b/av1-go_amd/host/av1_opstream.cpp
@@ -5,6 +5,7 @@
 #include <string>
 #include <vector>
 #include "../csrc/av1_ops_cdfs.hpp"
+#include "../csrc/av1_ops8.hpp"
 #include "av1_bitstream.hpp"
 
 namespace av1mi_host {
@@ -37,16 +38,6 @@
   if (n < 0) { if (err) *err = "tile payload overflow"; return false; }
   out->resize((size_t)n);
   return true;
-}
-template <int kBlocks>
-bool code_tile(const uint16_t *rec, int block_records, const int *nrec, const int *first, uint16_t *pos, int nslots, const uint16_t *total,
-               const uint16_t *base, int run, const av1ops::SlotTable &tab, const uint16_t *image, std::vector<uint8_t> *out, std::string *err) {
-  using namespace av1ops;
-  if (run > 65535) { if (err) *err = "tile too large for 16-bit entry positions"; return false; }
-  std::vector<op_t> list((size_t)first[kBlocks], 0);
-  std::vector<uint32_t> grouped((size_t)run, 0);
-  for (int b = 0; b < kBlocks; b++) replay_block<kBlocks>(rec + (size_t)b * block_records, nrec[b], pos, b, first[b], list.data(), grouped.data());
-  return code_list(list, grouped, nslots, total, base, tab, image, out, err);
 }
 struct WaveLoop {
   template <class T> using Var = av1ops::LaneVar<T, av1ops::kLanes32>;
@@ -93,7 +84,7 @@
   const size_t nb = (size_t)v.w8 * v.h8;
   std::vector<BlockInfo> info(nb);
   v.info = info.data();
-  for (size_t b = 0; b < nb; b++) { memset(&info[b], 0, sizeof(BlockInfo)); block_summary(v, (int)b, &info[b]); }
+  for (size_t b = 0; b < nb; b++) memset(&info[b], 0, sizeof(BlockInfo));
   if (!v.key) for (int r = 0; r < v.h8; r++) for (int c = 0; c < v.w8; c++) inter_mode_decision(v, r, c, &info[(size_t)r * v.w8 + c]);
   const int qcat = q_category(f.base_q_idx);
   SlotTable tab;
@@ -101,12 +92,11 @@
   const int sbr_n = (v.h8 + 7) / 8, sbc_n = (v.w8 + 7) / 8;
   tiles->assign((size_t)sbr_n * sbc_n, {});
   const int nslots = v.key ? S_KEY_END : S_INTER_END;
-  std::vector<uint8_t> cnt((size_t)S_MAX * kBlocksPerTile);
-  std::vector<uint16_t> pos((size_t)S_MAX * kBlocksPerTile), rec((size_t)kBlocksPerTile * kBlockRecords);
-  ScanTables scan;
-  fill_scan_tables(&scan);
-  alignas(16) uint8_t mag[kMagBytes];
-  const TokScratch ts = { mag, &scan };
+  std::vector<Tile8Mem> mem8(1);
+  std::vector<uint16_t> rec((size_t)kBlocksPerTile * kBlockRecords);
+  const uint32_t ops_cap8 = 1u << 20;
+  std::vector<op_t> list8(ops_cap8);
+  std::vector<uint32_t> grouped8(65536 + kListAlign);
   const bool stats = getenv("AV1MI_TOK_STATS") != nullptr;
   int st_rec = 0, st_cnt = 0, st_ops = 0, st_over = 0; long st_ops_sum = 0;
   SlotTable tab32;
@@ -126,35 +116,25 @@
         if (!code_list(list, grouped32, K_END, total, base, tab32, image32.data(), &(*tiles)[(size_t)sbr * sbc_n + sbc], err)) return false;
         continue;
       }
-      std::fill(cnt.begin(), cnt.end(), 0);
-      int first[kBlocksPerTile + 1], nrec[kBlocksPerTile];
-      first[0] = 0;
-      bool over = false;
-      for (int zi = 0; zi < kBlocksPerTile; zi++) {
-        Sink k = { &rec[(size_t)zi * kBlockRecords], cnt.data(), zi, 0, 0, false };
-        tok_block(v, k, ts, sbr, sbc, zi);
-        if (k.overflow && !stats) { if (err) *err = "a block exceeds the tokenizer's record area"; return false; }
-        over |= k.overflow;
-        nrec[zi] = k.nrec;
-        first[zi + 1] = first[zi] + k.n;
-        if (k.nrec > st_rec) st_rec = k.nrec;
+      WaveLoop wave;
+      uint16_t base[S_MAX], total[S_MAX];
+      const int words = tok_tile8(wave, mem8[0], v, sbr, sbc, rec.data(), list8.data(), ops_cap8, grouped8.data(), total, base);
+      if (stats) {
+        std::vector<uint8_t> cnt((size_t)S_MAX * kBlocksPerTile, 0);
+        const TokScratch ts = { mem8[0].p1.mag, &mem8[0].scan };
+        int ops = 0;
+        for (int zi = 0; zi < kBlocksPerTile; zi++) {
+          Sink k = { rec.data(), cnt.data(), zi, 0, 0, false };
+          tok_block(v, k, ts, sbr, sbc, zi, mem8[0].sums);
+          st_rec = std::max(st_rec, k.nrec); ops += k.n;
+        }
+        for (uint8_t c : cnt) st_cnt = std::max(st_cnt, (int)c);
+        st_ops = std::max(st_ops, ops); st_ops_sum += ops;
+        if (words < 0) { st_over++; continue; }
       }
-      if (stats) {
-        for (uint8_t c : cnt) if (c > st_cnt) st_cnt = c;
-        if (first[kBlocksPerTile] > st_ops) st_ops = first[kBlocksPerTile];
-        st_ops_sum += first[kBlocksPerTile];
-        if (over) { st_over++; continue; }
-      }
-      uint16_t base[S_MAX], total[S_MAX];
-      int run = 0;
-      for (int sl = 0; sl < nslots; sl++) {
-        const int n = group_positions(&cnt[(size_t)sl * kBlocksPerTile], &pos[(size_t)sl * kBlocksPerTile], run);
-        base[sl] = (uint16_t)run; total[sl] = (uint16_t)n;
-        run = (run + n + kListAlign - 1) & ~(kListAlign - 1);
-      }
-      if (!code_tile<kBlocksPerTile>(rec.data(), kBlockRecords, nrec, first, pos.data(), nslots, total, base, run, tab, image.data(),
-                                     &(*tiles)[(size_t)sbr * sbc_n + sbc], err))
-        return false;
+      if (words < 0) { if (err) *err = "a tile exceeds the tokenizer's capacities (records or symbols of a slot per block, entries per tile)"; return false; }
+      std::vector<op_t> list(list8.begin(), list8.begin() + words);
+      if (!code_list(list, grouped8, nslots, total, base, tab, image.data(), &(*tiles)[(size_t)sbr * sbc_n + sbc], err)) return false;
     }
   if (stats)
     fprintf(stderr, "[av1mi tok stats] %d tiles: records per block <= %d (capacity %d), symbols of a slot in a block <= %d (255), list words per tile <= %d, mean %.0f; %d tiles over a block capacity\n",
@@ -163,6 +143,24 @@
 }
 
 int opstream_slots() { return av1ops::S_MAX; }
+
+int opstream_tile8(const av1mi_obu_frame &f, int sbr, int sbc, uint32_t ops_cap, uint32_t *list, uint32_t *grouped, uint16_t *slot_total, uint16_t *slot_base,
+                   std::string *err) {
+  using namespace av1ops;
+  if (!opstream_supported(f, err) || sbr < 0 || sbc < 0 || sbr * 64 >= f.height || sbc * 64 >= f.width) return -2;
+  FrameView v;
+  frame_view_of(f, &v);
+  std::vector<uint8_t> zskip;
+  if (!v.key && !v.skip) { zskip.assign((size_t)v.w8 * v.h8, 0); v.skip = zskip.data(); }
+  if (!lr_units_of(f, &v, err)) return -2;
+  std::vector<BlockInfo> info(v.key ? 0 : (size_t)v.w8 * v.h8);
+  v.info = info.data();
+  if (!v.key) for (int r = 0; r < v.h8; r++) for (int c = 0; c < v.w8; c++) { memset(&info[(size_t)r * v.w8 + c], 0, sizeof(BlockInfo)); inter_mode_decision(v, r, c, &info[(size_t)r * v.w8 + c]); }
+  std::vector<Tile8Mem> mem(1);
+  std::vector<uint16_t> rec((size_t)kBlocksPerTile * kBlockRecords);
+  WaveLoop wave;
+  return tok_tile8(wave, mem[0], v, sbr, sbc, rec.data(), list, ops_cap, grouped, slot_total, slot_base);
+}
 
 int opstream_tile32(const av1mi_obu_frame &f, int sbr, int sbc, uint32_t ops_cap, uint32_t *list, uint32_t *grouped, uint16_t *slot_total, uint16_t *slot_base,
                     std::string *err) {
diff --git a/av1-go_amd/host/capi_host.cpp b/av1-go_amd/host/capi_host.cpp
--- a/av1-go_amd/host/capi_host.cpp
+++ b/av1-go_amd/host/capi_host.cpp
@@ -252,6 +252,12 @@
   std::string e;
   return av1::opstream_tile32(*f, sbr, sbc, ops_cap, list, grouped, slot_total, slot_base, &e);
 }
+int av1mi_host_opstream_tile8(const av1mi_obu_frame *f, int sbr, int sbc, uint32_t ops_cap, uint32_t *list, uint32_t *grouped, uint16_t *slot_total,
+                              uint16_t *slot_base) {
+  if (!f || !list || !grouped || !slot_total || !slot_base) return -2;
+  std::string e;
+  return av1::opstream_tile8(*f, sbr, sbc, ops_cap, list, grouped, slot_total, slot_base, &e);
+}
 long long av1mi_host_opstream_temporal_unit(const av1mi_obu_frame *f, int with_sequence_header, uint8_t *out, long long cap, char *err, int errcap) {
   return av1mi_host_opstream_key32_temporal_unit(f, 0, with_sequence_header, out, cap, err, errcap);
 }
```
